# enordber/pepr

Measured on AMD Instinct MI355X. Metric: M site-lnL/sec (WAG+G4 full-tree likelihood evaluations x alignment patterns); the gene-trees/sec half of BASELINE.json's metric is search.gene_trees_per_sec, higher is better.
Workload: dtype f64

## Files before the change

__graft_entry__.py:

```python
import os
import subprocess
import sys

ROOT = os.path.dirname(os.path.abspath(__file__))
if ROOT not in sys.path:
    sys.path.insert(0, ROOT)


def build_jni_double():
    d = os.path.join(ROOT, "tests", "jni_double")
    subprocess.check_call(["gcc", "-O2", "-fPIC", "-shared", "-Wall", "-Werror", "-I" + d, os.path.join(ROOT, "bindings", "jni", "peprml_jni.c"),
                           os.path.join(d, "jni_double.c"), "-L" + os.path.join(ROOT, "pepr_amd"), "-lpeprml",
                           "-Wl,-rpath," + os.path.join(ROOT, "pepr_amd"), "-o", os.path.join(d, "libjni_double.so")])


def build_kernel_harness():
    d = os.path.join(ROOT, "tests", "kernel_harness")
    rocm = os.environ.get("ROCM_PATH", "/opt/rocm")
    subprocess.check_call(["g++", "-O1", "-std=c++17", "-fPIC", "-shared", "-Wall", "-Werror", "-D__HIP_PLATFORM_AMD__", "-I" + os.path.join(rocm, "include"),
                           os.path.join(d, "kh.cpp"), "-L" + os.path.join(ROOT, "pepr_amd"), "-lpeprml", "-L" + os.path.join(rocm, "lib"), "-lamdhip64",
                           "-Wl,-rpath,$ORIGIN/../../pepr_amd", "-Wl,-rpath," + os.path.join(rocm, "lib"), "-o", os.path.join(d, "libkh.so")])


def build():
    subprocess.check_call(["make", "-s", "-C", os.path.join(ROOT, "pepr_amd", "csrc")])
    build_jni_double()
    build_kernel_harness()
    subprocess.check_call(["make", "-s", "-C", os.path.join(ROOT, "oracle")])
    try:
        head = subprocess.run(["git", "-C", ROOT, "rev-parse", "--short", "HEAD"], capture_output=True, text=True, timeout=10).stdout.strip()
        dirty = subprocess.run(["git", "-C", ROOT, "status", "--porcelain", "--untracked-files=no"], capture_output=True, text=True, timeout=10).stdout.strip()
        if head:
            with open(os.path.join(ROOT, "pepr_amd", "BUILD_COMMIT"), "w") as f:
                f.write(head + ("+dirty" if dirty else "") + "\n")
    except Exception:
        pass
    import pepr_amd
    from pepr_amd import _lib
    L = _lib.load()
    for s in _lib.SYMBOLS:
        assert hasattr(L, s), "missing symbol " + s


def smoke():
    import numpy as np
    from oracle import po
    from pepr_amd import engine, synth
    build_needed = not os.path.exists(os.path.join(ROOT, "pepr_amd", "libpeprml.so"))
    if build_needed:
        build()
    ctx = engine.Context(0)
    names, rows, nw = synth.simulate_alignment(12, 400, 7, missing_frac=0.2)
    r = ctx.score([(names, rows)], [nw], alpha=0.7, site_lnl=True)[0]
    a = po.Alignment(names, rows); t = po.Tree(nw, a); e = po.Engine(a, po.Model(0), 4, 0.7)
    ref, refs = e.site_lnl(t)
    assert abs(r["lnl"] - ref) < 1e-9 * abs(ref), (r["lnl"], ref)
    assert np.abs(r["site_lnl"] - refs).max() < 1e-9
    o = ctx.optimize([(names, rows)], [nw], alpha=1.0)[0]
    assert o["lnl"] >= r["lnl"] - 1e-6, (o["lnl"], r["lnl"])
    print("smoke ok: lnL %.6f (oracle %.6f), optimised %.6f alpha %.4f" % (r["lnl"], ref, o["lnl"], o["alpha"]))
    ctx.close()


if __name__ == "__main__":
    build()
    if len(sys.argv) > 1 and sys.argv[1] == "smoke":
        smoke()
```

pepr_amd/csrc/api.cpp:

```cpp
#include <algorithm>
#include <cstdlib>
#include <cstring>
#include <memory>
#include <new>
#include <thread>

#include "../../include/peprml.h"
#include "api_types.hpp"

using namespace pml;

static thread_local std::string g_err;

static std::mutex g_fp_mu; static unsigned g_fp_seen[16]; static int g_fp_n = 0;
void pml_fpguard::note(unsigned v) {
    v &= ~0x3Fu;
    std::lock_guard<std::mutex> lk(g_fp_mu);
    for (int i = 0; i < g_fp_n; ++i) if (g_fp_seen[i] == v) return;
    if (g_fp_n < 16) g_fp_seen[g_fp_n++] = v;
}

extern "C" {

const char *pml_version(void) { return "peprml 0.2 (gfx950)"; }
// ... 98 lines not shown
    if (!b || g < 0 || g >= (int)b->b.genes.size()) return PML_EINVAL;
    return b->b.genes[g].aln.npat;
}

#define LOCKED(b) std::lock_guard<std::mutex> lk((b)->owner->c.mu)
#define GUARD(expr)                                                                            \
    try { return (expr); }                                                                     \
    catch (const std::bad_alloc &) { return b->owner->c.fail(PML_ENOMEM, "host allocation failed"); } \
    catch (const std::exception &e) { return b->owner->c.fail(PML_EINVAL, e.what()); }

int pml_batch_score(pml_batch *b, double *lnl) {
    if (!b || !lnl) return PML_EINVAL;
    pml_fpguard fpg;
    LOCKED(b);
    GUARD(b->b.score(std::vector<char>(), lnl));
}
int pml_batch_score_stored(pml_batch *b, double *lnl) {
    if (!b || !lnl) return PML_EINVAL;
    pml_fpguard fpg;
    LOCKED(b);
    GUARD(b->b.score(std::vector<char>(), lnl, true));
}
int pml_batch_site_lnl(pml_batch *b, int g, double *out) {
    if (!b || !out || g < 0 || g >= (int)b->b.genes.size()) return PML_EINVAL;
    pml_fpguard fpg;
    LOCKED(b);
    GUARD(b->b.site_lnl(g, out));
}
int pml_batch_set_alpha(pml_batch *b, int g, double alpha) {
    if (!b || g >= (int)b->b.genes.size() || !(alpha > 0)) return PML_EINVAL;
    pml_fpguard fpg;
    LOCKED(b);
    if (g < 0) for (int i = 0; i < (int)b->b.genes.size(); ++i) b->b.set_alpha(i, alpha);
    else b->b.set_alpha(g, alpha);
    return PML_OK;
}
int pml_batch_root_derivs(pml_batch *b, double *lnl, double *d1, double *d2) {
    if (!b || !lnl || !d1 || !d2) return PML_EINVAL;
    pml_fpguard fpg;
    LOCKED(b);
    GUARD(b->b.root_derivs(lnl, d1, d2));
}
int pml_batch_optimize(pml_batch *b, const pml_search_opts *opts, double *lnl, double *alpha) {
    if (!b || !lnl) return PML_EINVAL;
    pml_fpguard fpg;
    LOCKED(b);
    const bool oa = opts ? opts->optimize_alpha != 0 : true;
    const double eps = (opts && opts->epsilon > 0) ? opts->epsilon : 1e-4;
    int rc;
    try { rc = b->b.optimize(oa, eps, lnl); }
    catch (const std::exception &e) { return b->owner->c.fail(PML_EINVAL, e.what()); }
    if (rc) return rc;
    if (alpha) for (size_t g = 0; g < b->b.genes.size(); ++g) alpha[g] = b->b.genes[g].alpha;
    return PML_OK;
}
int pml_batch_search(pml_batch *b, const pml_search_opts *opts, double *lnl, double *alpha) {
    if (!b || !lnl) return PML_EINVAL;
    pml_fpguard fpg;
    LOCKED(b);
    int rc;
    try { rc = opts ? b->b.set_constraints(opts->nconstraints, opts->constraint_ntax, opts->constraint_names, opts->constraint_rows) : 0;
          if (!rc) rc = b->b.search(opts ? opts->nni != 0 : true, opts ? opts->spr_radius : 0,
                           opts ? opts->optimize_alpha != 0 : true,
                           (opts && opts->epsilon > 0) ? opts->epsilon : 1e-3, lnl); }
    catch (const std::exception &e) { return b->owner->c.fail(PML_EINVAL, e.what()); }
    if (rc) return rc;
    if (alpha) for (size_t g = 0; g < b->b.genes.size(); ++g) alpha[g] = b->b.genes[g].alpha;
    return PML_OK;
}
int pml_batch_newick(pml_batch *b, int g, int digits, char **out) {
    if (!b || !out || g < 0 || g >= (int)b->b.genes.size()) return PML_EINVAL;
    pml_fpguard fpg;
    LOCKED(b);
    const Gene &G = b->b.genes[g];
    *out = dup_string(G.tree.newick(G.aln.names, digits));
    return *out ? PML_OK : PML_ENOMEM;
}

enum { OP_SCORE, OP_OPTIMIZE, OP_SEARCH };

static size_t gene_bytes_bound(const pml_alignment &a, bool score_only) {
    const size_t mp = ((size_t)std::max(a.nsites, 1) + 31) / 32 * 32, nt = (size_t)std::max(a.ntax, 3);
    const size_t slots = (score_only ? nt - 2 : 3 * (nt - 2)) + NSCRATCH + MAXTAIL;
    return slots * CLV_ROWS * ((mp + 127) / 128 * 128) * 8 + slots * mp * 4 + nt * mp + 64 * mp + (1 << 16);
}

static int oneshot_on(Ctx &c, int op, int n, const pml_alignment *alns, const char *const *newicks,
                      const pml_model *model, const pml_search_opts *opts, int flags, pml_result *const *out, int share) {
    pml_fpguard fpg;
    std::vector<std::string> pstart; std::vector<const char *> pnw;
    static_assert(sizeof(pml_alignment) == sizeof(pml_alignment_view), "alignment view layout");
    if (op == OP_SEARCH && opts && opts->seed != 0) {
        std::vector<int> idx;
        for (int i = 0; i < n; ++i) if (!newicks || !newicks[i]) idx.push_back(i);
        if (!idx.empty()) {
            std::vector<pml_alignment_view> views;
            for (int i : idx) views.push_back(pml_alignment_view{alns[i].ntax, alns[i].nsites, alns[i].names, alns[i].rows});
            std::vector<Tree> trees; std::vector<EncodedAlignment> enc; std::vector<long long> len; std::vector<int> moves;
            if (int prc = parsimony_batch(&c, (int)idx.size(), views.data(), opts->seed, 20, trees, enc, len, moves)) return prc;
            pstart.resize(n); pnw.assign(n, nullptr);
            for (int i = 0; i < n; ++i) if (newicks && newicks[i]) pnw[i] = newicks[i];
            for (size_t k = 0; k < idx.size(); ++k) { pstart[idx[k]] = trees[k].newick(enc[k].names, 6); pnw[idx[k]] = pstart[idx[k]].c_str(); }
            newicks = pnw.data();
        }
    }
    Batch b;
    struct Drop { Batch &b; ~Drop() { b.destroy(); } } drop{b};
    b.share = share;
    int rc;
    try {
        rc = b.create(&c, n, reinterpret_cast<const pml_alignment_view *>(alns), newicks, model ? model->pi_mode : PML_PI_RAXML_3DP,
                      model ? model->ncat : 4, model ? model->alpha : 1.0, op == OP_SCORE);
        if (rc) return rc;
        std::vector<double> lnl(n);
        if (op == OP_SCORE) rc = b.score(std::vector<char>(), lnl.data());
        else if (op == OP_OPTIMIZE)
            rc = b.optimize(opts ? opts->optimize_alpha != 0 : true, (opts && opts->epsilon > 0) ? opts->epsilon : 1e-4, lnl.data());
        else {
            rc = opts ? b.set_constraints(opts->nconstraints, opts->constraint_ntax, opts->constraint_names, opts->constraint_rows) : 0;
            if (!rc) rc = b.search(opts ? opts->nni != 0 : true, opts ? opts->spr_radius : 0, opts ? opts->optimize_alpha != 0 : true,
                                   (opts && opts->epsilon > 0) ? opts->epsilon : 1e-3, lnl.data());
        }
        for (int i = 0; i < n && !rc; ++i) {
            const Gene &G = b.genes[i];
            pml_result &r = *out[i];
            r.lnl = lnl[i]; r.alpha = G.alpha; r.tree_length = G.tree.length();
            r.npatterns = G.aln.npat; r.nsites = G.aln.nsites;
            r.newick = dup_string(G.tree.newick(G.aln.names, op == OP_SCORE ? 10 : 20));
            if (op == OP_SCORE && (flags & PML_WANT_SITE_LNL)) {
                r.site_lnl = (double *)std::malloc(sizeof(double) * (G.aln.nsites > 0 ? G.aln.nsites : 1));
                if (!r.site_lnl) rc = c.fail(PML_ENOMEM, "host allocation failed");
                else rc = b.site_lnl(i, r.site_lnl);
            }
        }
    } catch (const std::bad_alloc &) { rc = c.fail(PML_ENOMEM, "host allocation failed"); }
    catch (const std::exception &e) { rc = c.fail(PML_EINVAL, e.what()); }
    return rc;
}

static Ctx *worker_ctx(pml_ctx *ctx, int k) {
    while ((int)ctx->workers.size() <= k) {
        std::unique_ptr<Ctx> w(new Ctx());
        if (w->init_worker(ctx->c)) { ctx->c.last_error = w->last_error; return nullptr; }
        ctx->workers.push_back(std::move(w));
    }
    return ctx->workers[k].get();
}
static int search_groups(int n, const pml_alignment *alns) {
    static const int env = std::getenv("PML_GROUPS") ? std::atoi(std::getenv("PML_GROUPS")) : 0;
    int maxcols = 0;
    for (int i = 0; i < n; ++i) maxcols = std::max(maxcols, alns[i].nsites);
    const int tiles = (maxcols + 127) / 128;
    int g = env > 0 ? std::min(env, 8) : 2;
    if (env <= 0) { while (g > 1 && n / g < 32) --g; }
    if (!std::getenv("PML_GROUPS_FORCE")) { while (g > 1 && tiles * g > 32) --g; }
    return std::max(g, 1);
}

static int oneshot_chunk(pml_ctx *ctx, int op, int n, const pml_alignment *alns, const char *const *newicks,
                         const pml_model *model, const pml_search_opts *opts, int flags, pml_result *out) {
    const int G = (op == OP_SEARCH) ? search_groups(n, alns) : 1;
    if (G <= 1) {
        std::vector<pml_result *> outs(n);
        for (int i = 0; i < n; ++i) outs[i] = out + i;
        return oneshot_on(ctx->c, op, n, alns, newicks, model, opts, flags, outs.data(), 1);
    }
    for (int k = 0; k < G; ++k) if (!worker_ctx(ctx, k)) return PML_EDEVICE;
// ... 474 lines not shown
```

pepr_amd/csrc/engine.cpp:

```cpp
#include "engine.hpp"

#include <algorithm>
#include <atomic>
#include <chrono>
#include <cmath>
#include <thread>
#include <cstring>

namespace pml {

#define HIPCHK(expr)                                                                          \
    do {                                                                                      \
        hipError_t e_ = (expr);                                                               \
        if (e_ != hipSuccess)                                                                 \
            return ctx->fail(-5, std::string(#expr) + ": " + hipGetErrorString(e_));          \
    } while (0)

int Ctx::init(int dev, bool prof) {
    Ctx *ctx = this;
    int count = 0;
    if (hipGetDeviceCount(&count) != hipSuccess || count <= 0) return fail(-3, "no HIP device available");
    if (dev < 0 || dev >= count) return fail(-3, "device ordinal out of range");
    device = dev; profile = prof;
    HIPCHK(hipSetDevice(device));
// ... 37 lines not shown
}
static void fill_model_dev(const Model &m, ModelDev &h) {
    std::memcpy(h.eval, m.eval, sizeof h.eval);
    std::memcpy(h.U, m.U, sizeof h.U);
    std::memcpy(h.Uinv, m.Uinv, sizeof h.Uinv);
    std::memcpy(h.pi, m.pi, sizeof h.pi);
    for (int k = 0; k < NS; ++k) for (int j = 0; j < NS; ++j) h.UinvT[j * NS + k] = m.Uinv[k * NS + j];
}
const Matrix *Ctx::matrix_of(int pm) const {
    const Ctx &r = root ? *root : *this;
    if (pm < PM_REGISTERED || (size_t)(pm - PM_REGISTERED) / 2 >= r.matrices.size()) return nullptr;
    return &r.matrices[(size_t)(pm - PM_REGISTERED) / 2];
}
std::string Ctx::model_name(int pm) const {
    if (pm == 0) return "PROTGAMMAWAG";
    if (pm == 1) return "PROTGAMMAWAG (full-precision frequencies)";
    if (pm == 2) return "PROTGAMMAWAGF";
    if (pm == PM_GTR) return "PROTGAMMAGTR";
    const Matrix *m = matrix_of(pm);
    if (!m) return "model code " + std::to_string(pm);
    std::string n = "PROTGAMMA";
    for (char ch : m->name) n += (char)std::toupper((unsigned char)ch);
    return (pm & 1) ? n + "F" : n;
}
int Ctx::ensure_model(int pm) {
    Ctx *ctx = this;
    if (!valid_code(pm)) return fail(-1, "bad pi_mode " + std::to_string(pm) + " (not a built-in model and not a registered matrix)");
    if (model_per_gene(pm) || shared_of(pm)) return 0;
    Shared sh{pm, nullptr, nullptr};
    HIPCHK(hipSetDevice(device));
    HIPCHK(hipMalloc((void **)&sh.d_model, sizeof(ModelDev)));
    HIPCHK(hipMalloc((void **)&sh.d_eigfrags, sizeof(double) * 2 * PFRAG));
    if (const Matrix *M = matrix_of(pm)) {
        struct In { double exch[NEXCH], pi[NS]; ModelReq req; } h, *d = nullptr;
        std::memcpy(h.exch, M->exch, sizeof h.exch); std::memcpy(h.pi, M->pi, sizeof h.pi);
        HIPCHK(hipMalloc((void **)&d, sizeof(In)));
        h.req = ModelReq{d->exch, d->pi, sh.d_model, -1, 0.0};
        HIPCHK(hipMemcpy(d, &h, sizeof h, hipMemcpyHostToDevice));
        Ev ev = tic_self(K_MODEL, sizeof(ModelDev));
        launch_model_build(&d->req, 1, stream, ev.a, ev.b);
        if (int rc = sync(stream)) return rc;
        HIPCHK(hipFree(d));
    } else {
        Model m; m.init(pm);
        ModelDev h;
        fill_model_dev(m, h);
        HIPCHK(hipMemcpy(sh.d_model, &h, sizeof h, hipMemcpyHostToDevice));
    }
    launch_eigfrags(sh.d_model, sh.d_eigfrags, stream);
    if (int rc = sync(stream)) return rc;
    HIPCHK(hipGetLastError());
    shared.push_back(sh);
    return 0;
}

int Batch::alloc_gene_models() {
    const size_t n = genes.size();
    HIPCHK(hipMalloc((void **)&d_gmodel, n * sizeof(ModelDev)));
    HIPCHK(hipMalloc((void **)&d_geig, n * 2 * PFRAG * sizeof(double)));
    HIPCHK(hipMalloc((void **)&d_gexch, n * NEXCH * sizeof(double)));
    HIPCHK(hipMalloc((void **)&d_gpi, n * NS * sizeof(double)));
    HIPCHK(hipMalloc((void **)&d_mreq, n * sizeof(ModelReq)));
    HIPCHK(hipHostMalloc((void **)&h_gexch, n * NEXCH * sizeof(double), hipHostMallocDefault));
    HIPCHK(hipHostMalloc((void **)&h_gpi, n * NS * sizeof(double), hipHostMallocDefault));
    HIPCHK(hipHostMalloc((void **)&h_mreq, n * sizeof(ModelReq), hipHostMallocDefault));
    return 0;
}
void Batch::empirical_pi(int g, double *pi) const {
    if (genes[g].counted_pi.empty()) empirical_freqs(genes[g].aln, pi);
    else std::memcpy(pi, genes[g].counted_pi.data(), sizeof(double) * NS);
}
void Batch::matrix_for(int g, double *exch, double *pi) const {
    const int code = genes[g].model_code;
    const Matrix *M = ctx->matrix_of(code);
    std::memcpy(exch, M ? M->exch : wag_exch(), sizeof(double) * NEXCH);
    if (code == PM_GTR) { const double last = exch[NEXCH - 1]; for (int i = 0; i < NEXCH; ++i) exch[i] /= last; }
    if (model_per_gene(code)) empirical_pi(g, pi);
    else std::memcpy(pi, M ? M->pi : wag_pi(code), sizeof(double) * NS);
    double sum = 0;
    for (int i = 0; i < NS; ++i) sum += pi[i];
    for (int i = 0; i < NS; ++i) pi[i] /= sum;
}
int Batch::build_gene_models() {
    const int n = (int)genes.size();
    if (int rc = alloc_gene_models()) return rc;
    std::vector<ModelDev> h(n);
    std::vector<int> dev;
    for (int g = 0; g < n; ++g) {
        const int code = genes[g].model_code;
        if (code == 2) {
            double pi[NS];
            empirical_pi(g, pi);
            Model m; m.init_pi(pi);
            fill_model_dev(m, h[g]);
            std::memcpy(h_gexch + (size_t)g * NEXCH, wag_exch(), sizeof(double) * NEXCH); std::memcpy(h_gpi + (size_t)g * NS, m.pi, sizeof m.pi);
            HIPCHK(hipMemcpyAsync(d_gmodel + g, &h[g], sizeof(ModelDev), hipMemcpyHostToDevice, ctx->stream));
            continue;
        }
        matrix_for(g, h_gexch + (size_t)g * NEXCH, h_gpi + (size_t)g * NS);
        if (model_per_gene(code)) { dev.push_back(g); continue; }
        if (int rc = ctx->ensure_model(code)) return rc;
        HIPCHK(hipMemcpyAsync(d_gmodel + g, ctx->shared_of(code)->d_model, sizeof(ModelDev), hipMemcpyDeviceToDevice, ctx->stream));
    }
    HIPCHK(hipMemcpyAsync(d_gexch, h_gexch, (size_t)n * NEXCH * sizeof(double), hipMemcpyHostToDevice, ctx->stream));
    HIPCHK(hipMemcpyAsync(d_gpi, h_gpi, (size_t)n * NS * sizeof(double), hipMemcpyHostToDevice, ctx->stream));
    if (int rc = build_models(dev, -1, nullptr)) return rc;
    if (dev.empty()) launch_eigfrags_n(d_gmodel, d_geig, n, ctx->stream);
    if (int rc = ctx->sync(ctx->stream)) return rc;
    HIPCHK(hipGetLastError());
    return 0;
}
int Batch::build_models(const std::vector<int> &gs, int patch, const double *vals) {
    if (gs.empty()) return 0;
    static const bool host_arm = std::getenv("PML_MODEL_HOST") != nullptr;
    const int n = (int)genes.size(), m = (int)gs.size();
    if (host_arm) {
        if (!h_gmodel) HIPCHK(hipHostMalloc((void **)&h_gmodel, (size_t)n * sizeof(ModelDev), hipHostMallocDefault));
        for (int i = 0; i < m; ++i) {
            const int g = gs[i];
            double ex[NEXCH];
            std::memcpy(ex, h_gexch + (size_t)g * NEXCH, sizeof ex);
            if (patch >= 0) ex[patch] = vals[i];
            Model md; md.init(ex, h_gpi + (size_t)g * NS);
            fill_model_dev(md, h_gmodel[g]);
            HIPCHK(hipMemcpyAsync(d_gmodel + g, h_gmodel + g, sizeof(ModelDev), hipMemcpyHostToDevice, ctx->stream));
        }
    } else {
        for (int i = 0; i < m; ++i) {
            const int g = gs[i];
            h_mreq[i] = ModelReq{d_gexch + (size_t)g * NEXCH, d_gpi + (size_t)g * NS, d_gmodel + g, patch, patch >= 0 ? vals[i] : 0.0};
        }
        HIPCHK(hipMemcpyAsync(d_mreq, h_mreq, (size_t)m * sizeof(ModelReq), hipMemcpyHostToDevice, ctx->stream));
        Ctx::Ev ev = ctx->tic_self(K_MODEL, (double)m * sizeof(ModelDev));
        launch_model_build(d_mreq, m, ctx->stream, ev.a, ev.b);
    }
    launch_eigfrags_n(d_gmodel, d_geig, n, ctx->stream);
    return 0;
}
int Batch::set_matrix(int g, const double *exch, const double *pi) {
    const int n = (int)genes.size();
    HIPCHK(hipSetDevice(ctx->device));
    if (!d_gmodel) {
        if (int rc = alloc_gene_models()) return rc;
        for (int i = 0; i < n; ++i) {
            matrix_for(i, h_gexch + (size_t)i * NEXCH, h_gpi + (size_t)i * NS);
            HIPCHK(hipMemcpyAsync(d_gmodel + i, d_shared, sizeof(ModelDev), hipMemcpyDeviceToDevice, ctx->stream));
            HIPCHK(hipMemcpyAsync(d_geig + (size_t)i * 2 * PFRAG, d_shared_eig, sizeof(double) * 2 * PFRAG, hipMemcpyDeviceToDevice, ctx->stream));
        }
        plan.valid = false;
    }
    std::vector<int> gs;
    for (int i = 0; i < n; ++i) if (g < 0 || i == g) gs.push_back(i);
    for (int i : gs) {
        std::memcpy(h_gexch + (size_t)i * NEXCH, exch, sizeof(double) * NEXCH);
        if (pi) {
            double sum = 0;
            for (int k = 0; k < NS; ++k) sum += pi[k];
            for (int k = 0; k < NS; ++k) h_gpi[(size_t)i * NS + k] = pi[k] / sum;
        }
        invalidate_all(i);
    }
    HIPCHK(hipMemcpyAsync(d_gexch, h_gexch, (size_t)n * NEXCH * sizeof(double), hipMemcpyHostToDevice, ctx->stream));
    HIPCHK(hipMemcpyAsync(d_gpi, h_gpi, (size_t)n * NS * sizeof(double), hipMemcpyHostToDevice, ctx->stream));
    if (int rc = build_models(gs, -1, nullptr)) return rc;
    if (int rc = ctx->sync(ctx->stream)) return rc;
    HIPCHK(hipGetLastError());
    return 0;
}
int Batch::get_matrix(int g, double *exch, double *pi) const {
    if (h_gexch) {
        if (exch) std::memcpy(exch, h_gexch + (size_t)g * NEXCH, sizeof(double) * NEXCH);
        if (pi) std::memcpy(pi, h_gpi + (size_t)g * NS, sizeof(double) * NS);
        return 0;
    }
    double ex[NEXCH], p[NS];
    matrix_for(g, ex, p);
    if (exch) std::memcpy(exch, ex, sizeof ex);
    if (pi) std::memcpy(pi, p, sizeof p);
    return 0;
}
hipEvent_t Ctx::get_event() {
    if (!pool.empty()) { hipEvent_t e = pool.back(); pool.pop_back(); return e; }
    hipEvent_t e; hipEventCreate(&e); return e;
}
void Ctx::tic(int kind, double bytes, double flops) {
    stats[kind].launches++; stats[kind].bytes += bytes; stats[kind].flops += flops;
    if (!profile) return;
    Ev ev{kind, get_event(), get_event()};
    hipEventRecord(ev.a, tic_stream ? tic_stream : stream);
    pending.push_back(ev);
}
void Ctx::toc() {
    if (!profile) return;
    hipEventRecord(pending.back().b, tic_stream ? tic_stream : stream);
}
Ctx::Ev Ctx::tic_self(int kind, double bytes, double flops) {
    stats[kind].launches++; stats[kind].bytes += bytes; stats[kind].flops += flops;
    if (!profile) return Ev{kind, nullptr, nullptr};
    pending.push_back(Ev{kind, get_event(), get_event()});
    return pending.back();
}
void Ctx::resolve_events() {
    for (auto &e : pending) {
        float ms = 0;
        if (hipEventElapsedTime(&ms, e.a, e.b) == hipSuccess) stats[e.kind].ms += ms;
        pool.push_back(e.a); pool.push_back(e.b);
    }
    pending.clear();
}

static size_t align_up(size_t x, size_t a) { return (x + a - 1) / a * a; }

struct DetRec { int batch, ntax, npat, nsites, kind, a, b, pad; double x, y, z; };
static std::vector<DetRec> *g_det = nullptr;
static std::mutex g_det_mu;
static bool det_on() {
    static const bool on = [] {
        const char *p = std::getenv("PML_DET_LOG");
        if (!p) return false;
        g_det = new std::vector<DetRec>(); g_det->reserve(1 << 22);
        std::atexit([] {
            const char *q = std::getenv("PML_DET_LOG"); FILE *f = q ? std::fopen(q, "w") : nullptr;
            if (!f) return;
            for (const DetRec &r : *g_det) std::fprintf(f, "B%d g%d_%d_%d %c %d %d %a %a %a\n", r.batch, r.ntax, r.npat, r.nsites, (char)r.kind, r.a, r.b, r.x, r.y, r.z);
            std::fclose(f);
        });
        return true;
    }();
    return on;
}
void det_record(int batch, const Gene &G, char kind, int a, int b, double x, double y, double z) {
    if (!det_on()) return;
    std::lock_guard<std::mutex> lk(g_det_mu);
    g_det->push_back(DetRec{batch, G.aln.ntax, G.aln.npat, G.aln.nsites, kind, a, b, 0, x, y, z});
}
static std::atomic<int> g_batch_id{0};
static double now_ms();

int Batch::create(Ctx *c, int n, const pml_alignment_view *alns, const char *const *newicks, int pm, int nc,
                  double alpha, bool score_only, const int *gene_codes) {
    ctx = c; pi_mode = pm; ncat = nc; score_only_batch = score_only;
    det_id = ++g_batch_id;
    virtual_cherries = std::getenv("PML_NO_CHERRY") == nullptr;
    virtual_pitch = virtual_cherries && std::getenv("PML_NO_PITCH") == nullptr;
    if (n <= 0) return ctx->fail(-1, "empty batch");
    if (nc != 1 && nc != 4) return ctx->fail(-1, "ncat must be 1 or 4");
    if (gene_codes) { for (int g = 0; g < n; ++g) if (!ctx->valid_code(gene_codes[g])) return ctx->fail(-1, "bad pi_mode " + std::to_string(gene_codes[g])); }
    else if (int rc = ctx->ensure_model(pm)) return rc;
    const bool per_gene = gene_codes != nullptr || model_per_gene(pm);
    if (!per_gene) { d_shared = ctx->shared_of(pm)->d_model; d_shared_eig = ctx->shared_of(pm)->d_eigfrags; }
    HIPCHK(hipSetDevice(ctx->device));
    genes.resize(n);
    for (int g = 0; g < n; ++g) genes[g].model_code = gene_codes ? gene_codes[g] : pm;
    const double t_create0 = now_ms();
    {
        const int nthreads = std::max(1, std::min({n, 16, (int)std::thread::hardware_concurrency()}));
        std::vector<std::string> errs(n);
        std::atomic<int> next{0};
        auto work = [&]() {
            for (int g = next++; g < n; g = next++) {
                Gene &G = genes[g];
                try {
                    if (!G.aln.encode(alns[g].ntax, alns[g].nsites, alns[g].names, alns[g].rows, errs[g])) continue;
                    if (newicks && newicks[g]) { if (!Tree::parse(newicks[g], G.aln.names, G.tree, errs[g])) continue; }
                    else G.tree = nj_tree(G.aln);
                } catch (const std::exception &e) { errs[g] = e.what(); }
            }
        };
        std::vector<std::thread> pool;
        for (int t = 1; t < nthreads; ++t) pool.emplace_back(work);
        work();
        for (auto &t : pool) t.join();
        for (int g = 0; g < n; ++g) if (!errs[g].empty()) return ctx->fail(-2, "gene " + std::to_string(g) + ": " + errs[g]);
    }
    if (std::getenv("PML_TRACE")) fprintf(stderr, "[pml] create: encode + start trees of %d genes %.1f ms\n", n, now_ms() - t_create0);
    if (int rc = layout(alpha, score_only)) return rc;
    return per_gene ? build_gene_models() : 0;
}

int Batch::layout(double alpha, bool score_only) {
    const int n = (int)genes.size();
    size_t total = 0;
    std::vector<size_t> off(n);
    for (int g = 0; g < n; ++g) {
        Gene &G = genes[g];
        const int nt = G.aln.ntax, mp = G.aln.mpad, ndir = 3 * (nt - 2);
        G.slot_cap = score_only ? (nt - 2) : ndir;
        G.slot_of.assign(ndir, -1); G.valid.assign(ndir, 0); G.pend_level.assign(ndir, -1);
        G.mark_all();
        off[g] = total;
        total += align_up((size_t)nt * mp, 256);
        total += align_up((size_t)mp * 8, 256);
        total += (size_t)(G.slot_cap + NSCRATCH) * clv_doubles(mp) * 8;
        total += align_up((size_t)(G.slot_cap + NSCRATCH) * mp * 4, 256);
        total += (size_t)MAXTAIL * clv_doubles(mp) * 8;
        total += (size_t)MAXTAIL * align_up((size_t)mp * 4, 256);
        total += (size_t)MAXTAIL * align_up((size_t)mp * 8, 256);
    }
    arena_bytes = total;
    const double t_alloc0 = now_ms();
    if (ctx->arena_cache && ctx->arena_cache_bytes >= total) {
        arena = ctx->arena_cache; arena_bytes = ctx->arena_cache_bytes;
        ctx->arena_cache = nullptr; ctx->arena_cache_bytes = 0;
    } else {
        if (ctx->arena_cache) { hipFree(ctx->arena_cache); ctx->arena_cache = nullptr; ctx->arena_cache_bytes = 0; }
        if (hipMalloc((void **)&arena, total) != hipSuccess) {
            arena = nullptr;
            return ctx->fail(-4, "device arena of " + std::to_string(total >> 20) + " MiB does not fit");
        }
    }
    if (std::getenv("PML_POISON_ARENA")) HIPCHK(hipMemsetAsync(arena, 0xFF, total, ctx->stream));
    for (int g = 0; g < n; ++g) {
        Gene &G = genes[g];
        const int nt = G.aln.ntax, mp = G.aln.mpad;
        char *p = arena + off[g];
        G.d_codes = (uint8_t *)p; p += align_up((size_t)nt * mp, 256);
        G.d_weight = (double *)p; p += align_up((size_t)mp * 8, 256);
        G.d_clv = (double *)p; p += (size_t)(G.slot_cap + NSCRATCH) * clv_doubles(mp) * 8;
        G.d_scl = (int *)p; p += align_up((size_t)(G.slot_cap + NSCRATCH) * mp * 4, 256);
        for (int k = 0; k < MAXTAIL; ++k) { G.d_sumtab[k] = (double *)p; p += clv_doubles(mp) * 8; }
        for (int k = 0; k < MAXTAIL; ++k) { G.d_sumscl[k] = (int *)p; p += align_up((size_t)mp * 4, 256); }
        for (int k = 0; k < MAXTAIL; ++k) { G.d_patlnl[k] = (double *)p; p += align_up((size_t)mp * 8, 256); }
        if (!G.aln.codes.empty()) {
            HIPCHK(hipMemcpyAsync(G.d_codes, G.aln.codes.data(), (size_t)nt * mp, hipMemcpyHostToDevice, ctx->stream));
            HIPCHK(hipMemcpyAsync(G.d_weight, G.aln.weight.data(), (size_t)mp * 8, hipMemcpyHostToDevice, ctx->stream));
        }
        set_alpha(g, alpha);
    }
    scalars_doubles = (size_t)8 * MAXTAIL * n;
    HIPCHK(hipMalloc((void **)&d_scalars, sizeof(double) * scalars_doubles));
    HIPCHK(hipHostMalloc((void **)&h_scalars, sizeof(double) * scalars_doubles, hipHostMallocDefault));
    std::memset(h_scalars, 0, sizeof(double) * scalars_doubles);
    HIPCHK(hipHostMalloc((void **)&h_plan_lnl, sizeof(double) * n, hipHostMallocMapped | hipHostMallocCoherent));
    HIPCHK(hipHostGetDevicePointer((void **)&d_plan_lnl, h_plan_lnl, 0));
    { if (int rc_ = ctx->sync(ctx->stream)) return rc_; }
    if (std::getenv("PML_TRACE")) fprintf(stderr, "[pml] layout: arena %.1f GiB allocated + uploaded in %.1f ms\n", (double)total / (1 << 30), now_ms() - t_alloc0);
    return 0;
}

void Batch::destroy() {
    if (!ctx) return;
    hipSetDevice(ctx->device);
    if (arena) {
        if (ctx->arena_cache_bytes < arena_bytes) {
            if (ctx->arena_cache) hipFree(ctx->arena_cache);
            ctx->arena_cache = arena; ctx->arena_cache_bytes = arena_bytes;
        } else hipFree(arena);
    }
    if (h_stage) hipHostFree(h_stage);
    if (d_stage) hipFree(d_stage);
    if (d_frags) hipFree(d_frags);
    if (d_nsync) hipFree(d_nsync);
    if (d_nctl) {
        if (std::getenv("PML_TRACE")) {
            NewtonCtl h[2];
            if (hipMemcpy(h, d_nctl, sizeof h, hipMemcpyDeviceToHost) == hipSuccess && h[0].n_requests)
                fprintf(stderr, "[pml] branch Newton: %llu requests, %.2f evaluations each\n", h[0].n_requests, (double)h[0].n_evals / (double)h[0].n_requests);
        }
        hipFree(d_nctl); d_nctl = nullptr;
    }
    if (d_gmodel) { hipFree(d_gmodel); d_gmodel = nullptr; }
    if (d_geig) { hipFree(d_geig); d_geig = nullptr; }
    if (d_gexch) { hipFree(d_gexch); d_gexch = nullptr; }
    if (d_gpi) { hipFree(d_gpi); d_gpi = nullptr; }
    if (d_mreq) { hipFree(d_mreq); d_mreq = nullptr; }
    if (h_gexch) { hipHostFree(h_gexch); h_gexch = nullptr; }
    if (h_gpi) { hipHostFree(h_gpi); h_gpi = nullptr; }
    if (h_mreq) { hipHostFree(h_mreq); h_mreq = nullptr; }
    if (h_gmodel) { hipHostFree(h_gmodel); h_gmodel = nullptr; }
    if (ev_stagger) { hipEventDestroy(ev_stagger); ev_stagger = nullptr; }
    if (d_nsync2) hipFree(d_nsync2);
    if (d_frags2) hipFree(d_frags2);
    d_nsync = d_nsync2 = nullptr; d_frags2 = nullptr; nsync_cap = nsync_cap2 = 0; frag_cap2 = 0;
    if (plan.h) hipHostFree(plan.h);
    if (plan.d) hipFree(plan.d);
    plan = Plan();
    if (h_scalars) hipHostFree(h_scalars);
    if (d_scalars) hipFree(d_scalars);
    if (h_plan_lnl) hipHostFree(h_plan_lnl);
    h_plan_lnl = d_plan_lnl = nullptr;
    if (h_chain) hipHostFree(h_chain);
    if (d_chain) hipFree(d_chain);
    if (d_lenpool) hipFree(d_lenpool);
    if (d_tailpool) { hipFree(d_tailpool); d_tailpool = nullptr; tailpool_cap = 0; }
    if (d_site2pat) { hipFree(d_site2pat); d_site2pat = nullptr; }
    h_chain = d_chain = nullptr; d_lenpool = nullptr; chain_cap = 0;
    arena = nullptr; h_stage = d_stage = nullptr; d_frags = nullptr; d_scalars = h_scalars = nullptr;
}

int GeneStore::create(Ctx *c, int n, const pml_alignment_view *alns) {
    ctx = c;
    HIPCHK(hipSetDevice(ctx->device));
    items.resize(n);
    std::vector<std::string> errs(n);
    std::atomic<int> next{0};
    auto work = [&]() {
        for (int g = next++; g < n; g = next++) {
            try { if (items[g].aln.encode(alns[g].ntax, alns[g].nsites, alns[g].names, alns[g].rows, errs[g])) pair_counts(items[g].aln, items[g].cmp, items[g].diff); }
            catch (const std::exception &e) { errs[g] = e.what(); }
        }
    };
    const int nthreads = std::max(1, std::min({n, 16, (int)std::thread::hardware_concurrency()}));
    std::vector<std::thread> pool;
    for (int t = 1; t < nthreads; ++t) pool.emplace_back(work);
    work();
    for (auto &t : pool) t.join();
    for (int g = 0; g < n; ++g) if (!errs[g].empty()) return ctx->fail(-2, "gene " + std::to_string(g) + ": " + errs[g]);
    size_t total = 0;
    for (auto &it : items) total += align_up((size_t)it.aln.ntax * it.aln.mpad, 256) + align_up((size_t)it.aln.mpad * 8, 256);
    if (hipMalloc((void **)&arena, total) != hipSuccess) { arena = nullptr; return ctx->fail(-4, "gene store does not fit on the device"); }
    char *p = arena;
    for (auto &it : items) {
        it.d_codes = (uint8_t *)p; p += align_up((size_t)it.aln.ntax * it.aln.mpad, 256);
        it.d_w = (double *)p; p += align_up((size_t)it.aln.mpad * 8, 256);
        HIPCHK(hipMemcpyAsync(it.d_codes, it.aln.codes.data(), (size_t)it.aln.ntax * it.aln.mpad, hipMemcpyHostToDevice, ctx->stream));
        HIPCHK(hipMemcpyAsync(it.d_w, it.aln.weight.data(), (size_t)it.aln.mpad * 8, hipMemcpyHostToDevice, ctx->stream));
    }
    { if (int rc_ = ctx->sync(ctx->stream)) return rc_; }
    return 0;
}
void GeneStore::destroy() { if (arena) { hipSetDevice(ctx->device); hipFree(arena); arena = nullptr; } items.clear(); }

int Batch::create_replicates(Ctx *c, const GeneStore &store, const std::vector<std::vector<int>> &sel, int pm, int nc, double alpha) {
    ctx = c; pi_mode = pm; ncat = nc; score_only_batch = false;
    virtual_cherries = std::getenv("PML_NO_CHERRY") == nullptr;
    virtual_pitch = virtual_cherries && std::getenv("PML_NO_PITCH") == nullptr;
    const int n = (int)sel.size();
    if (n <= 0) return ctx->fail(-1, "empty batch");
    if (int rc = ctx->ensure_model(pm)) return rc;
    const bool per_gene = model_per_gene(pm);
    if (!per_gene) { d_shared = ctx->shared_of(pm)->d_model; d_shared_eig = ctx->shared_of(pm)->d_eigfrags; }
    HIPCHK(hipSetDevice(ctx->device));
    genes.resize(n);
    for (auto &G : genes) G.model_code = pm;
    struct SegH { int rep, gene, off; size_t rowmap_off; };
    std::vector<SegH> segs; std::vector<int> rowmaps;
    int max_npat = 0;
    for (int r = 0; r < n; ++r) {
        Gene &G = genes[r]; EncodedAlignment &A = G.aln;
        std::vector<std::string> names;
// ... 223 lines not shown
    Gene &G = genes[g];
    const int nt = G.aln.ntax;
    if (v < nt || virt_kind(g, v, to)) return 0;
    {
        const int idx0 = (v - nt) * 3 + G.tree.slot(v, to);
        if (G.valid[idx0]) return 0;
        if (G.pend_level[idx0] >= 0) return G.pend_level[idx0];
    }
    struct Frame { int v, to, k, stage, lv[2]; };
    std::vector<Frame> st;
    st.reserve(64);
    st.push_back({v, to, G.tree.slot(v, to), 0, {0, 0}});
    int ret = 0;
    while (!st.empty()) {
        Frame &f = st.back();
        const int idx = (f.v - nt) * 3 + f.k;
        if (f.stage == 0) {
            if (G.valid[idx]) { ret = 0; st.pop_back(); continue; }
            if (G.pend_level[idx] >= 0) { ret = G.pend_level[idx]; st.pop_back(); continue; }
        }
        int ch[2], ci = 0;
        for (int q = 0; q < 3; ++q) if (q != f.k) ch[ci++] = G.tree.nbr[f.v][q];
        if (f.stage >= 1) f.lv[f.stage - 1] = ret;
        if (f.stage < 2) {
            const int c = ch[f.stage];
            f.stage++;
            if (c < nt || virt_kind(g, c, f.v)) { ret = 0; continue; }
            const int fv = f.v;
            st.push_back({c, fv, G.tree.slot(c, fv), 0, {0, 0}});
            continue;
        }
        const int lvl = std::max(f.lv[0], f.lv[1]) + 1;
        PendingOp op; op.gene = g; op.out_kind = SIDE_MSG; op.out_id = idx; op.level = lvl; ci = 0;
        for (int q = 0; q < 3; ++q) if (q != f.k) { op.child[ci] = msg(g, G.tree.nbr[f.v][q], f.v); op.t[ci] = G.tree.len[f.v][q]; ci++; }
        ops.push_back(op);
        G.pend_level[idx] = lvl;
        ret = lvl;
        st.pop_back();
    }
    return ret;
}

static double now_ms() {
    return std::chrono::duration<double, std::milli>(std::chrono::steady_clock::now().time_since_epoch()).count();
}

void Batch::newton_gave_up() {
    ++ctx->newton_giveups;
    if (std::getenv("PML_TRACE") && d_nctl) {
        NewtonCtl h[2];
        if (hipMemcpy(h, d_nctl, sizeof h, hipMemcpyDeviceToHost) == hipSuccess)
            fprintf(stderr, "[pml] k_newton exchange gave up: slice %d of %d, evaluation %d, arrived mask %08x%08x, tickets taken in its partition %d, (left * 1024 + partition) %d; tickets %d %d done %d %d oticket %d %d %d %d %d %d %d %d odone %d\n",
                    h[0].dbg[1], h[0].dbg[2], h[0].dbg[3], (unsigned)h[0].dbg[5], (unsigned)h[0].dbg[4], (unsigned)h[0].dbg[6], h[0].dbg[7], h[0].ticket[0], h[0].ticket[1], h[0].done[0], h[0].done[1],
                    h[0].oticket[0], h[0].oticket[1], h[0].oticket[2], h[0].oticket[3], h[0].oticket[4], h[0].oticket[5], h[0].oticket[6], h[0].oticket[7], h[0].odone);
        hipMemset(&d_nctl[0].dbg[0], 0, sizeof(int));
    }
    safe_left = safe_hold; safe_hold = std::min(safe_hold * 2, 1024);
}
int Batch::clear_abort() {
    if (!d_nctl) return 0;
    for (int l = 0; l < 2; ++l) HIPCHK(hipMemsetAsync(&d_nctl[l].abort, 0, sizeof(int), l ? ctx->stream2 : ctx->stream));
    { if (int rc_ = ctx->sync(ctx->stream2)) return rc_; }
    { if (int rc_ = ctx->sync(ctx->stream)) return rc_; }
    return 0;
}

int Batch::flush_deferred() {
    if (deferred.empty()) return 0;
    struct Guard { Batch *b; ~Guard() { b->deferred.clear(); b->ctx->tic_stream = nullptr; } } guard{this};
    const size_t lo = deferred.front().base, hi = deferred.back().base + deferred.back().bytes;
    const hipStream_t cs = deferred.front().lane ? ctx->stream2 : ctx->stream;
    HIPCHK(hipMemcpyAsync((char *)d_stage + lo, (char *)h_stage + lo, hi - lo, hipMemcpyHostToDevice, cs));
    const ModelDev *md = d_gmodel ? nullptr : d_shared;
    static const bool serialize = std::getenv("PML_SERIALIZE") != nullptr;
#define PML_SER() do { if (serialize) hipStreamSynchronize(st); } while (0)
    if (serialize) hipStreamSynchronize(cs);
    for (const Deferred &L : deferred) {
        const hipStream_t st = L.lane ? ctx->stream2 : ctx->stream;
        double *const frags_buf = L.lane ? d_frags2 : d_frags;
        char *ds = (char *)d_stage + L.base;
        ctx->tic_stream = st;
        if (L.nreq) {
            ctx->tic(K_PMAT, (double)L.nreq * PFRAG * 8);
            launch_pmat(md, (const PmatReq *)(ds + L.o_req), frags_buf, (int)L.nreq, st, d_gmodel != nullptr);
            ctx->toc(); PML_SER();
        }
        if (L.nruns) {
            ctx->tic(K_NEWVIEW, L.algo_bytes, L.algo_flops);
            launch_oplist((const NvOp *)(ds + L.o_ops), (const GeneRun *)(ds + L.o_runs), (int)L.nruns, L.max_mpad, L.any_pitch, L.any_chain, st, L.fused ? d_nctl + L.lane : nullptr);
            ctx->toc(); PML_SER();
        }
        if (L.stagger) hipEventRecord(ev_stagger, st);
        if (L.neval) {
            ctx->tic(K_REDUCE, 0);
            launch_reduce((const ReduceReq *)(ds + L.o_red), (int)L.neval, st);
            ctx->toc(); PML_SER();
        }
        if (L.nt_reg + L.nt_stream > 0) {
            ctx->tic(K_NEWTON, L.newton_bytes);
            if (L.seq) { launch_newton_seq(md, (const NewtonReq *)(ds + L.o_newt), (const int *)(ds + L.o_tick), L.nt_reg, L.nt_stream, d_nctl + L.lane, st); ++ctx->newton_seq_launches; }
            else launch_newton(md, (const NewtonReq *)(ds + L.o_newt), (const int *)(ds + L.o_tick), L.nt_reg, L.nt_stream, d_nctl + L.lane, st);
            ctx->toc(); PML_SER();
        }
        ctx->tic_stream = nullptr;
        if (hipError_t e = hipGetLastError(); e != hipSuccess) return ctx->fail(-5, std::string("kernel launch: ") + hipGetErrorString(e));
    }
#undef PML_SER
    flush_quota = std::min<size_t>(flush_quota * 2, 8);
    return 0;
}

int Batch::run(std::vector<PendingOp> &ops, const std::vector<Tail> &tails) {
    const double t_begin = now_ms();
    HIPCHK(hipSetDevice(ctx->device));
    std::stable_sort(ops.begin(), ops.end(), [](const PendingOp &a, const PendingOp &b) { return a.gene != b.gene ? a.gene < b.gene : a.part < b.part; });
    const size_t nops = ops.size(), ntail = tails.size();
    size_t neval = 0, nnewton = 0;
    for (auto &t : tails) { if (t.mode == MODE_EVALUATE) neval++; else if (t.mode != MODE_EVALUATE_CAT) nnewton++; }
    size_t nreq_max = 10 * nops + 9 * ntail;
    {
        std::vector<char> seen(genes.size(), 0);
        size_t keyed = 0, loose = 0;
        for (auto &o : ops) { if (!seen[o.gene]) { seen[o.gene] = 1; keyed += 5 * (size_t)genes[o.gene].aln.ntax; }
                              if (o.out_kind != SIDE_MSG) loose += (o.bv[0] < 0) + (o.bv[1] < 0); }
        for (auto &t : tails) { if (!seen[t.gene]) { seen[t.gene] = 1; keyed += 5 * (size_t)genes[t.gene].aln.ntax; }
                                if (t.mode >= MODE_EVALUATE && t.bv < 0) loose += 1; }
        nreq_max = std::min(nreq_max, keyed + loose);
    }
    bool any_pitch = false, any_chain = false;
    if (int rc = ensure_frags(std::max(nreq_max, (size_t)1))) return rc;
    double *&nsync_buf = lane ? d_nsync2 : d_nsync; size_t &nsync_c = lane ? nsync_cap2 : nsync_cap;
    if (nnewton > nsync_c) {
        if (chain) { if (int rc = chain_sync()) return rc; }
        if (nsync_buf) hipFree(nsync_buf);
        nsync_buf = nullptr; nsync_c = 0;
        const size_t cap = std::max(nnewton * 2, (size_t)256);
        HIPCHK(hipMalloc((void **)&nsync_buf, cap * NEWTON_SYNC_DOUBLES * sizeof(double)));
        HIPCHK(hipMemsetAsync(nsync_buf, 0, cap * NEWTON_SYNC_DOUBLES * sizeof(double), ctx->stream));
        { if (int rc_ = ctx->sync(ctx->stream)) return rc_; }
        nsync_c = cap;
    }
    if (nnewton && !d_nctl) {
        HIPCHK(hipMalloc((void **)&d_nctl, 2 * sizeof(NewtonCtl)));
        HIPCHK(hipMemsetAsync(d_nctl, 0, 2 * sizeof(NewtonCtl), ctx->stream));
        { if (int rc_ = ctx->sync(ctx->stream)) return rc_; }
    }
    const hipStream_t st = lane ? ctx->stream2 : ctx->stream;
    double *const frags_buf = lane ? d_frags2 : d_frags;
    ctx->tic_stream = st;
    const size_t ngenes = genes.size();
    std::vector<int> &nparts = run_nparts; nparts.assign(ngenes, 1);
    for (auto &o : ops) nparts[o.gene] = std::max(nparts[o.gene], o.part + 1);
    for (auto &t : tails) nparts[t.gene] = std::max(nparts[t.gene], t.part + 1);
    std::vector<size_t> &koff = run_koff; koff.assign(ngenes + 1, 0);
    for (size_t g = 0; g < ngenes; ++g) koff[g + 1] = koff[g] + (size_t)nparts[g];
    const size_t nkeys = koff[ngenes];
    const size_t o_req = 0;
    const size_t o_ops = align_up(o_req + nreq_max * sizeof(PmatReq), 256);
    const size_t o_runs = align_up(o_ops + (nops + ntail) * sizeof(NvOp), 256);
    const size_t o_red = align_up(o_runs + nkeys * sizeof(GeneRun), 256);
    const size_t o_newt = align_up(o_red + neval * sizeof(ReduceReq), 256);
    size_t ntick_max = 0;
    for (auto &t : tails) if (t.mode == MODE_SUMTABLE) ntick_max += (size_t)newton_split(genes[t.gene].aln.mpad);
    const size_t o_tick = align_up(o_newt + nnewton * sizeof(NewtonReq), 256);
    const size_t bytes = align_up(o_tick + ntick_max * sizeof(int), 256);
    if (chain && chain_off + bytes > h_cap) { if (int rc = chain_sync()) return rc; }
    if (int rc = ensure_stage(bytes)) return rc;
    const size_t base = chain ? chain_off : 0;
    if (chain) chain_off += bytes;
    char *hs = (char *)h_stage + base, *ds = (char *)d_stage + base;
    PmatReq *hreq = (PmatReq *)(hs + o_req);
    NvOp *hops = (NvOp *)(hs + o_ops);
    GeneRun *hruns = (GeneRun *)(hs + o_runs);
    ReduceReq *hred = (ReduceReq *)(hs + o_red);
    NewtonReq *hnewt = (NewtonReq *)(hs + o_newt);
    int *htick = (int *)(hs + o_tick);
    if (nnewton) ++newton_launch_seq;
    const unsigned tag_base = (newton_launch_seq & 0x3FFFFFu) << 10;
    static const bool fuse_env = std::getenv("PML_NO_FUSE") == nullptr && !(std::getenv("PML_CHAIN") && std::atoi(std::getenv("PML_CHAIN")) == 0);
    const bool fuse_ok = fuse_env && !newton_safe_mode();
    std::vector<char> fused_req(nnewton, 0);
    bool any_fused = false;
    std::vector<int> tail_req(ntail, -1);

    size_t nout = 0, nruns = 0, ie = 0, in = 0, ireq = 0, iop = 0;
    last_src.clear();
    int max_mpad = 0, newton_maxm = 0;
    double algo_bytes = 0, algo_flops = 0;
    bool req_ok = req_off.size() == genes.size() + 1;
    for (size_t g = 0; req_ok && g < genes.size(); ++g) req_ok = req_off[g + 1] - req_off[g] == (size_t)9 * genes[g].tree.nnodes();
    if (!req_ok) {
        req_off.assign(genes.size() + 1, 0);
        for (size_t g = 0; g < genes.size(); ++g) req_off[g + 1] = req_off[g] + (size_t)3 * 3 * genes[g].tree.nnodes();
        req_stamp.assign(req_off.back(), 0); req_ptr.assign(req_off.back(), nullptr); req_launch = 0;
        val_bucket.assign(genes.size() * 3, {}); val_stamp.assign(genes.size() * 3, 0);
    }
    if (++req_launch == 0) {
        std::fill(req_stamp.begin(), req_stamp.end(), 0u); std::fill(val_stamp.begin(), val_stamp.end(), 0u); req_launch = 1;
    }
    bool req_overflow = false;
    auto add_req = [&](size_t g, double t, int kind, int v, int q) -> const double * {
        uint64_t tbits = 0; size_t key = 0;
        std::vector<std::pair<uint64_t, const double *>> *bucket = nullptr;
        if (!record_plan) {
            if (v >= 0) {
                const Tree &T = genes[g].tree;
                const int w = T.nbr[v][q], a = v * 3 + q, b = w * 3 + T.slot(w, v);
                key = req_off[g] + (size_t)kind * 3 * T.nnodes() + (size_t)std::min(a, b);
                if (req_stamp[key] == req_launch) return req_ptr[key];
            } else {
                std::memcpy(&tbits, &t, 8);
                const size_t bi = g * 3 + (size_t)kind;
                if (val_stamp[bi] != req_launch) { val_bucket[bi].clear(); val_stamp[bi] = req_launch; }
                bucket = &val_bucket[bi];
                for (auto &e : *bucket) if (e.first == tbits) return e.second;
            }
        }
        if (ireq >= nreq_max) { req_overflow = true; return frags_buf; }
        PmatReq &r = hreq[ireq];
        r.t = t; std::memcpy(r.rates, genes[g].rates, sizeof r.rates); r.kind = kind; r.pad = 0;
        r.tp = (chain && v >= 0 && genes[g].len_pending[(size_t)v * 3 + q]) ? genes[g].d_len + (size_t)v * 3 + q : nullptr;
        r.md = d_gmodel ? d_gmodel + g : nullptr;
        last_src.push_back({(int)g, v, q, kind});
        const double *out = frags_buf + (ireq++) * FRAG_STRIDE;
        if (!record_plan) { if (v >= 0) { req_stamp[key] = req_launch; req_ptr[key] = out; } else bucket->push_back({tbits, out}); }
        return out;
    };
    struct Resolved { OpSide s; int kind; const int *scl; double bytes; double flops = 0; bool inner = true; };
    auto resolve = [&](size_t g, const Side &sd, Resolved &R) -> int {
        Gene &G = genes[g];
        const int mp = G.aln.mpad, nt = G.aln.ntax;
        R.s = OpSide{nullptr, nullptr, nullptr, nullptr, nullptr, nullptr, nullptr}; R.scl = nullptr;
        R.flops = 0; R.inner = true;
        if (sd.kind == SIDE_TIP) { R.kind = SK_TIP; R.s.p0 = G.d_codes + (size_t)sd.id * mp; R.bytes = 1; R.inner = false; return 0; }
        if (sd.kind == SIDE_CHERRY) {
            const int v = nt + sd.id / 3, k = sd.id % 3;
            int tips[2], qs[2], ci = 0;
            for (int q = 0; q < 3; ++q) if (q != k) { tips[ci] = G.tree.nbr[v][q]; qs[ci] = q; ++ci; }
            R.kind = SK_CHERRY;
            R.s.p0 = G.d_codes + (size_t)tips[0] * mp; R.s.p1 = G.d_codes + (size_t)tips[1] * mp;
            R.s.t0 = add_req(g, G.tree.len[v][qs[0]], PM_TIPTABLE, v, qs[0]);
            R.s.t1 = add_req(g, G.tree.len[v][qs[1]], PM_TIPTABLE, v, qs[1]);
            R.bytes = 640 + 642;
            R.flops = 80;
            return 0;
        }
        if (sd.kind == SIDE_PITCH) {
            const int X = nt + sd.id / 3, k = sd.id % 3;
            int qc = -1, qC = -1;
            for (int q = 0; q < 3; ++q) if (q != k) { if (G.tree.nbr[X][q] < nt) qc = q; else qC = q; }
            const int C = G.tree.nbr[X][qC], kC = G.tree.slot(C, X);
            int tips[2], qs[2], ci = 0;
            for (int q = 0; q < 3; ++q) if (q != kC) { tips[ci] = G.tree.nbr[C][q]; qs[ci] = q; ++ci; }
            R.kind = SK_PITCH;
            R.s.p0 = G.d_codes + (size_t)tips[0] * mp; R.s.p1 = G.d_codes + (size_t)tips[1] * mp;
            R.s.p2 = G.d_codes + (size_t)G.tree.nbr[X][qc] * mp;
            R.s.t0 = add_req(g, G.tree.len[C][qs[0]], PM_TIPTABLE, C, qs[0]);
            R.s.t1 = add_req(g, G.tree.len[C][qs[1]], PM_TIPTABLE, C, qs[1]);
            R.s.t2 = add_req(g, G.tree.len[X][qc], PM_TIPTABLE, X, qc);
            R.s.f = add_req(g, G.tree.len[X][qC], PM_FRAGS, X, qC);
            any_pitch = true;
            R.bytes = 640 + (640 + 642) + 1 + 640;
            R.flops = 80 + 3280;
            return 0;
        }
        const int slot = sd.kind == SIDE_MSG ? G.slot_of[sd.id] : G.slot_cap + sd.id;
        if (slot < 0) return -1;
        R.kind = SK_CLV; R.s.p0 = G.d_clv + (size_t)slot * clv_doubles(mp); R.scl = G.d_scl + (size_t)slot * mp; R.bytes = 640;
        return 0;
    };

    std::vector<std::vector<int>> &tails_of = run_tails_of;
    if (tails_of.size() < nkeys) tails_of.resize(nkeys);
    for (auto &v : tails_of) v.clear();
    for (size_t i = 0; i < ntail; ++i) {
        if (tails[i].slot < 0 || tails[i].slot >= MAXTAIL) return ctx->fail(-1, "internal: bad tail slot");
        tails_of[koff[tails[i].gene] + (size_t)tails[i].part].push_back((int)i);
    }
    for (size_t g = 0; g < ngenes; ++g) for (int part = 0; part < nparts[g]; ++part) {
        const size_t key = koff[g] + (size_t)part;
        const bool has_ops = iop < nops && ops[iop].gene == (int)g && ops[iop].part == part;
        if (!has_ops && tails_of[key].empty()) continue;
        Gene &G = genes[g];
        const int mp = G.aln.mpad;
        GeneRun &run = hruns[nruns++];
        run.op_begin = (int)nout;
        max_mpad = std::max(max_mpad, mp);
        static const int chain_env = std::getenv("PML_CHAIN") ? std::atoi(std::getenv("PML_CHAIN")) : 2;
        const bool chain_reads = chain_env == 2 || (chain_env == 1 && record_plan), chain_nostore = chain_env >= 1 && record_plan && !record_stored;
        long last_nv = -1, last_nv_op = -1;
        auto chained_from = [&](const Side &sd, int kind) {
            return chain_reads && last_nv >= 0 && kind == SK_CLV && sd.kind == ops[last_nv_op].out_kind && sd.id == ops[last_nv_op].out_id;
        };
        auto consume_last = [&]() {
            any_chain = true;
            if (chain_nostore || ops[last_nv_op].transient) { hops[last_nv].flags |= OPF_NO_STORE; ops[last_nv_op].unstored = true; }
        };
        auto emit_tail = [&](const Tail &t) -> int {
            NvOp &d = hops[nout++];
            std::memset(&d, 0, sizeof d);
            Resolved L, R;
            if (resolve(g, t.a, L) || resolve(g, t.b, R)) return ctx->fail(-5, "internal: tail message has no slot");
            d.l = L.s; d.r = R.s; d.l_scl = L.scl; d.r_scl = R.scl;
            d.flags = L.kind | (R.kind << 2); d.mpad = mp; d.mode = t.mode;
            if (chained_from(t.a, L.kind)) { d.flags |= OPF_CHAIN_L; consume_last(); }
            else if (t.mode >= MODE_EVALUATE && chained_from(t.b, R.kind)) { d.flags |= OPF_CHAIN_R; consume_last(); }
            double *result = t.result_dev ? t.result_dev : d_scalars + 8 * (g * MAXTAIL + t.slot);
            if (t.mode == MODE_EVALUATE_CAT) {
                if (!t.patlnl_dev || !t.scl_dev) return ctx->fail(-1, "internal: table slice missing");
                d.pl = d.pr = add_req(g, t.t0, PM_FRAGS_PI, t.bv, t.bq);
                d.out = t.patlnl_dev; d.out_scl = t.scl_dev;
                algo_bytes += (double)G.aln.npat * (L.bytes + R.bytes + 36);
                algo_flops += (double)G.aln.npat * (3360 + L.flops + R.flops);
            } else if (t.mode == MODE_EVALUATE) {
                d.pl = d.pr = add_req(g, t.t0, PM_FRAGS_PI, t.bv, t.bq);
                double *pl = t.patlnl_dev ? t.patlnl_dev : G.d_patlnl[t.slot];
                d.out = pl; d.out_scl = nullptr;
                ReduceReq &rr = hred[ie++];
                rr.patlnl = pl; rr.weight = G.d_weight; rr.out = result; rr.mpad = mp; rr.pad = 0;
                algo_bytes += (double)G.aln.npat * (L.bytes + R.bytes + 8);
                algo_flops += (double)G.aln.npat * (3360 + L.flops + R.flops);
            } else {
                d.pl = eig_of((int)g); d.pr = d.pl + PFRAG;
                double *stab = t.sumtab_dev ? t.sumtab_dev : G.d_sumtab[t.slot];
                int *sscl = t.sumtab_dev ? reinterpret_cast<int *>(t.sumtab_dev + clv_doubles(mp)) : G.d_sumscl[t.slot];
                d.out = stab; d.out_scl = sscl;
                NewtonReq &nr = hnewt[in];
                nr.md = model_of((int)g); nr.tag_base = tag_base; nr.pad0 = 0;
                if (fuse_ok && !t.patlnl_dev && newton_reg_form(mp)) {
                    d.flags |= OPF_FUSED_NEWTON; d.aux = (const NewtonReq *)(ds + o_newt) + in;
                    fused_req[in] = 1; any_fused = true; any_chain = true;
                }
                last_nv = -1; last_nv_op = -1;
                tail_req[&t - tails.data()] = (int)in;
                nr.ticket0 = 0; nr.pad = 0;
                nr.sumtab = stab; nr.weight = G.d_weight; nr.scl = sscl;
                std::memcpy(nr.rates, G.rates, sizeof nr.rates);
                nr.t0 = t.t0; nr.tol = newton_tol; nr.out = result; nr.mpad = mp; nr.max_iter = t.max_iter;
                nr.t_dev0 = t.t_dev0; nr.t_dev1 = t.t_dev1; nr.patlnl = t.patlnl_dev;
                nr.sync = nsync_buf + (size_t)in * NEWTON_SYNC_DOUBLES; newton_maxm = std::max(newton_maxm, mp);
                algo_bytes += (double)G.aln.npat * (L.bytes + R.bytes + 640);
                algo_flops += (double)G.aln.npat * (6480 + L.flops + R.flops);
                in++;
            }
            return 0;
        };
        size_t ti = 0; int emitted = 0;
        auto flush_tails = [&](bool all) -> int {
            while (ti < tails_of[key].size()) {
                const Tail &t = tails[tails_of[key][ti]];
                if (!all && (t.after < 0 || t.after > emitted)) break;
                if (int rc = emit_tail(t)) return rc;
                ++ti;
            }
            return 0;
        };
        if (int rc = flush_tails(false)) return rc;
        for (; iop < nops && ops[iop].gene == (int)g && ops[iop].part == part; ++iop) {
            PendingOp &o = ops[iop];
            const int s = o.out_kind == SIDE_MSG ? slot_for(G, o.out_id) : G.slot_cap + o.out_id;
            if (s < 0) return ctx->fail(-4, "CLV slots exhausted (score-only batch used for a multi-root request)");
            NvOp &d = hops[nout++];
            std::memset(&d, 0, sizeof d);
            d.mode = MODE_NEWVIEW;
            d.out = G.d_clv + (size_t)s * clv_doubles(mp);
            d.out_scl = G.d_scl + (size_t)s * mp;
            Resolved S[2];
            if (resolve(g, o.child[0], S[0]) || resolve(g, o.child[1], S[1])) return ctx->fail(-5, "internal: child message has no slot");
            d.mpad = mp;
            d.flags = S[0].kind | (S[1].kind << 2);
            const double *pm[2];
            for (int c = 0; c < 2; ++c) {
                int bv = o.bv[c], bq = o.bq[c];
                if (o.out_kind == SIDE_MSG) {
                    bv = G.aln.ntax + o.out_id / 3; const int k = o.out_id % 3;
                    int seen = 0;
                    for (bq = 0; bq < 3; ++bq) if (bq != k) { if (seen == c) break; ++seen; }
                }
                pm[c] = add_req(g, o.t[c], PM_FRAGS, bv, bq);
            }
            Side ch[2] = {o.child[0], o.child[1]};
            if (chained_from(ch[1], S[1].kind)) { std::swap(S[0], S[1]); std::swap(pm[0], pm[1]); std::swap(ch[0], ch[1]); }
            d.flags = S[0].kind | (S[1].kind << 2);
            if (chained_from(ch[0], S[0].kind)) { d.flags |= OPF_CHAIN_L; consume_last(); }
            d.l = S[0].s; d.r = S[1].s; d.l_scl = S[0].scl; d.r_scl = S[1].scl; d.pl = pm[0]; d.pr = pm[1];
            algo_bytes += (double)G.aln.npat * (S[0].bytes + S[1].bytes + 640);
            algo_flops += (double)G.aln.npat * ((S[0].inner && S[1].inner ? 6480 : (S[0].inner || S[1].inner ? 3280 : 80)) + S[0].flops + S[1].flops);
            last_nv = (long)nout - 1; last_nv_op = (long)iop;
            ++emitted;
            if (int rc = flush_tails(false)) return rc;
        }
        if (int rc = flush_tails(true)) return rc;
        run.op_end = (int)nout;
        if (mp <= 16 * TILE_PAT)
            for (int i = run.op_begin; i < run.op_end; ++i) if (hops[i].mode == MODE_NEWVIEW) hops[i].flags |= OPF_NT_STORE;
    }

    if (req_overflow) return ctx->fail(-5, "internal: transition-matrix request bound exceeded");
    int nt_reg = 0, nt_stream = 0;
    const bool seq_launch = nnewton > 0 && newton_safe_mode();
    {
        int cur = 0;
        for (int pass = 0; pass < 2; ++pass) {
            for (size_t i = 0; i < nnewton; ++i) {
                if (fused_req[i] || newton_reg_form(hnewt[i].mpad) != (pass == 0)) continue;
                const int S = seq_launch ? 1 : newton_split(hnewt[i].mpad);
                hnewt[i].ticket0 = cur - (pass == 0 ? 0 : nt_reg);
                for (int k = 0; k < S; ++k) htick[cur++] = (int)i;
            }
            if (pass == 0) nt_reg = cur; else nt_stream = cur - nt_reg;
        }
        if (nnewton && safe_left > 0 && !safe_now) --safe_left;
    }
    double newton_bytes = 0;
    for (size_t i = 0; i < ntail; ++i) if (tails[i].mode == MODE_SUMTABLE && !fused_req[tail_req[i]]) newton_bytes += (double)genes[tails[i].gene].aln.npat * 640;
    Deferred L;
    L.base = base; L.bytes = bytes; L.o_req = o_req; L.o_ops = o_ops; L.o_runs = o_runs; L.o_red = o_red; L.o_newt = o_newt;
    L.o_tick = o_tick; L.nt_reg = nt_reg; L.nt_stream = nt_stream; L.seq = seq_launch; L.fused = any_fused;
    L.nreq = ireq; L.nruns = nruns; L.neval = neval; L.nnewton = nnewton; L.max_mpad = max_mpad; L.newton_maxm = newton_maxm;
    L.any_pitch = any_pitch; L.any_chain = any_chain; L.algo_bytes = algo_bytes; L.algo_flops = algo_flops; L.newton_bytes = newton_bytes; L.lane = lane; L.stagger = record_stagger;
    record_stagger = false;
    deferred.push_back(L);
    const bool defer = chain && !lanes_active;
    if (!defer || deferred.size() >= flush_quota) { if (int rc = flush_deferred()) return rc; }
    ctx->tic_stream = nullptr;
    const double t_launched = now_ms();
    ctx->stats[K_HOST_BUILD].launches++; ctx->stats[K_HOST_BUILD].ms += t_launched - t_begin;
    if (!chain) {
        bool pooled = false;
        for (auto &t : tails) pooled = pooled || t.result_host != nullptr;
        if (int rc = fetch_results(pooled)) return rc;
        { if (int rc_ = ctx->sync(ctx->stream)) return rc_; }
        HIPCHK(hipGetLastError());
        const double t_done = now_ms();
        ctx->stats[K_HOST_WAIT].launches++; ctx->stats[K_HOST_WAIT].ms += t_done - t_launched;
        host_phase_ms[HP_RUN_SYNCED] += t_launched - t_begin;
        ctx->resolve_events();
        auto result_of = [&](const Tail &t) { return t.result_host ? t.result_host : (t.result_dev ? (const double *)nullptr : res(t.gene, t.slot)); };
        std::vector<int> bad;
        for (size_t i = 0; i < ntail; ++i) {
            const Tail &t = tails[i];
            if (t.mode != MODE_SUMTABLE) continue;
            const double *h = result_of(t);
            if (h && !std::isfinite(h[1])) bad.push_back(tail_req[i]);
        }
        bool bad_fused = false;
        for (int i : bad) bad_fused = bad_fused || fused_req[i];
        if (bad_fused && !in_retry) {
            newton_gave_up(); ctx->newton_reissued += (long long)bad.size();
            if (int rc = clear_abort()) return rc;
            for (auto &o : ops) { o.unstored = false; if (o.out_kind == SIDE_MSG) genes[o.gene].pend_level[o.out_id] = -1; }
            in_retry = true;
            const int rc = run(ops, tails);
            in_retry = false;
            return rc;
        }
        if (!bad.empty() && !seq_launch && !bad_fused) {
            newton_gave_up(); ctx->newton_reissued += (long long)bad.size();
            int nr = 0, ns = 0;
            for (int pass = 0; pass < 2; ++pass) for (int i : bad) if (newton_reg_form(hnewt[i].mpad) == (pass == 0)) { htick[nr + ns] = i; ++(pass == 0 ? nr : ns); }
            if (int rc = clear_abort()) return rc;
            HIPCHK(hipMemcpyAsync(ds + o_tick, hs + o_tick, bad.size() * sizeof(int), hipMemcpyHostToDevice, ctx->stream));
            launch_newton_seq(nullptr, (const NewtonReq *)(ds + o_newt), (const int *)(ds + o_tick), nr, ns, d_nctl + lane, ctx->stream);
            ++ctx->newton_seq_launches;
            if (int rc = fetch_results(pooled)) return rc;
            { if (int rc_ = ctx->sync(ctx->stream)) return rc_; }
            HIPCHK(hipGetLastError());
        }
        for (auto &t : tails) {
            if (t.mode == MODE_EVALUATE_CAT) continue;
            const double *h = result_of(t);
#ifndef ABL_KEEP_GOING
            if (h && !std::isfinite(t.mode == MODE_EVALUATE ? h[0] : h[1]))
                return ctx->fail(-5, t.mode == MODE_EVALUATE ? "device returned a non-finite likelihood" : "k_newton: non-finite branch likelihood (also from the no-exchange form)");
#endif
        }
    }
    for (auto &o : ops) if (o.out_kind == SIDE_MSG) { Gene &G = genes[o.gene]; G.valid[o.out_id] = o.unstored ? 0 : 1; G.pend_level[o.out_id] = -1; }
    if (record_plan) {
        record_plan = false;
        Plan &P = plan;
        if (P.bytes < bytes) {
            if (P.h) hipHostFree(P.h);
            if (P.d) hipFree(P.d);
            P.h = P.d = nullptr; P.bytes = 0;
            HIPCHK(hipHostMalloc(&P.h, bytes)); HIPCHK(hipMalloc(&P.d, bytes)); P.bytes = bytes;
        }
        std::memcpy(P.h, hs, bytes);
        HIPCHK(hipMemcpyAsync(P.d, ds, bytes, hipMemcpyDeviceToDevice, ctx->stream));
        ReduceReq *pred = (ReduceReq *)((char *)P.h + o_red);
        P.per_gene = neval == genes.size();
        for (size_t g = 0; P.per_gene && g < neval; ++g) P.per_gene = pred[g].out == d_scalars + 8 * (g * MAXTAIL);
        if (P.per_gene) {
            for (size_t g = 0; g < neval; ++g) pred[g].out = d_plan_lnl + g;
            HIPCHK(hipMemcpyAsync((char *)P.d + o_red, pred, neval * sizeof(ReduceReq), hipMemcpyHostToDevice, ctx->stream));
        }
        P.len_seen.assign(genes.size(), {});
        P.o_req = o_req; P.o_ops = o_ops; P.o_runs = o_runs; P.o_red = o_red;
        P.nreq = ireq; P.nruns = nruns; P.neval = neval; P.max_mpad = max_mpad; P.algo_bytes = algo_bytes; P.algo_flops = algo_flops; P.stored = record_stored; P.any_pitch = any_pitch; P.any_chain = any_chain;
        P.rates_seen.resize(genes.size()); for (size_t g = 0; g < genes.size(); ++g) P.rates_seen[g] = genes[g].rates_epoch;
        P.src = last_src; P.outs.clear();
// ... 87 lines not shown
}
int Batch::site_lnl(int g, double *out) {
    Gene &G = genes[g];
    if ((int)G.aln.site2pat.size() != G.aln.nsites) return ctx->fail(-1, "per-site lnL is not available for device-gathered replicates");
    std::vector<char> act(genes.size(), 0); act[g] = 1;
    std::vector<double> l(genes.size());
    if (int rc = evaluate(act, l.data())) return rc;
    std::vector<double> pat(G.aln.mpad);
    HIPCHK(hipMemcpy(pat.data(), G.d_patlnl[0], sizeof(double) * G.aln.mpad, hipMemcpyDeviceToHost));
    for (int s = 0; s < G.aln.nsites; ++s) out[s] = pat[G.aln.site2pat[s]];
    return 0;
}
int Batch::root_derivs(double *lnl, double *d1, double *d2) {
    std::vector<PendingOp> ops; std::vector<Tail> tails;
    for (int g = 0; g < (int)genes.size(); ++g) {
        Gene &G = genes[g];
        const int r = G.tree.nbr[0][0];
        need(g, r, 0, ops);
        tails.push_back({g, msg(g, 0, r), msg(g, r, 0), MODE_SUMTABLE, G.tree.len[0][0], 0});
    }
    if (int rc = run(ops, tails)) return rc;
    for (int g = 0; g < (int)genes.size(); ++g) { lnl[g] = res(g)[1]; d1[g] = res(g)[2]; d2[g] = res(g)[3]; }
    return 0;
}

int Batch::smooth_pass(const std::vector<char> &active, std::vector<double> &maxdelta, double thr) {
    const int n = (int)genes.size();
    maxdelta.assign(n, 0.0);
    struct SafeOff { bool &f; ~SafeOff() { f = false; } } safe_off{safe_now};
    double hp_t = now_ms();
    std::vector<std::vector<std::pair<int, int>>> &order = pass_order;
    std::vector<std::vector<uint8_t>> &next = pass_next;
    if ((int)order.size() != n) { order.assign(n, {}); next.assign(n, {}); }
    size_t maxlen = 0;
    struct F { int v, from, k; };
    std::vector<F> st; st.reserve(256);
    for (int g = 0; g < n; ++g) {
        order[g].clear();
        if (!active[g]) { next[g].clear(); continue; }
        Gene &G = genes[g];
        const Tree &T = G.tree; const int nt = T.ntax;
        if (G.dirty.size() != (size_t)T.nnodes() * 3) G.mark_all();
        next[g].assign((size_t)T.nnodes() * 3, 0);
        st.clear(); st.push_back({0, -1, 0});
        while (!st.empty()) {
            F &f = st.back();
            if (f.k >= 3) { st.pop_back(); continue; }
            const int k = f.k, w = T.nbr[f.v][k]; f.k++;
            if (w < 0 || w == f.from) continue;
            if (G.dirty[f.v * 3 + k]) order[g].push_back({f.v, w});
            if (w >= nt) { const int fv = f.v; st.push_back({w, fv, 0}); }
        }
        maxlen = std::max(maxlen, order[g].size());
    }
    ++cnt_passes;
    host_phase_ms[HP_PASS_SETUP] += now_ms() - hp_t; hp_t = now_ms();
    static const bool no_chain = std::getenv("PML_NO_CHAIN") != nullptr;
    size_t nres = 0; for (int g = 0; g < n; ++g) nres += order[g].size();
    struct Done { int gene, v, w; double old; size_t idx; };
    std::vector<Done> done; done.reserve(nres);
    for (int attempt = 0; attempt < 2; ++attempt) {
    done.clear();
    if (!no_chain) { if (int rc = chain_begin(nres)) return rc; }
    auto fail_out = [&](int rc) { if (chain) { chain_sync(); chain = false; } return rc; };
    static const bool lanes_on = std::getenv("PML_LANES") != nullptr;
    int nact = 0; for (int g = 0; g < n; ++g) nact += active[g] && !order[g].empty();
    const bool two_lanes = chain && lanes_on && nact >= 16;
    lanes_active = two_lanes;
    for (size_t step = 0; step < maxlen; ++step) {
        ++cnt_smooth;
        const size_t first = done.size();
        for (int ln = 0; ln < (two_lanes ? 2 : 1); ++ln) {
            std::vector<PendingOp> ops; std::vector<Tail> tails;
            for (int g = 0; g < n; ++g) {
                if (!active[g] || step >= order[g].size()) continue;
                if (two_lanes && (g & 1) != ln) continue;
                auto [v, w] = order[g][step];
                Gene &G = genes[g];
                need(g, v, w, ops); need(g, w, v, ops);
                Tail t{g, msg(g, v, w), msg(g, w, v), MODE_SUMTABLE, G.tree.len[v][G.tree.slot(v, w)], 32};
                if (chain) {
                    t.result_dev = d_chain + 4 * done.size();
                    t.t_dev0 = G.d_len + (size_t)v * 3 + G.tree.slot(v, w); t.t_dev1 = G.d_len + (size_t)w * 3 + G.tree.slot(w, v);
                }
                done.push_back({g, v, w, t.t0, done.size()});
                tails.push_back(t);
            }
            if (tails.empty()) continue;
            lane = ln;
            if (two_lanes && step == 0) {
                if (!ev_stagger) hipEventCreateWithFlags(&ev_stagger, hipEventDisableTiming);
                if (ln == 0) record_stagger = true;
                else hipStreamWaitEvent(ctx->stream2, ev_stagger, 0);
            }
            const int rc = run(ops, tails);
            lane = 0;
            if (rc) return fail_out(rc);
        }
        if (chain) {
            for (size_t i = first; i < done.size(); ++i) {
                Gene &G = genes[done[i].gene]; const int v = done[i].v, w = done[i].w;
                G.len_pending[(size_t)v * 3 + G.tree.slot(v, w)] = 1; G.len_pending[(size_t)w * 3 + G.tree.slot(w, v)] = 1;
                branch_changed(done[i].gene, v, w);
            }
        } else {
            for (size_t i = first; i < done.size(); ++i) {
                Gene &G = genes[done[i].gene]; const int v = done[i].v, w = done[i].w;
                const double nl = res(done[i].gene)[0], old = done[i].old, dl = std::fabs(nl - old);
                maxdelta[done[i].gene] = std::max(maxdelta[done[i].gene], dl);
                if (nl != old) { G.tree.set_len(v, w, nl); branch_changed(done[i].gene, v, w); }
                if (dl > thr) { std::swap(G.dirty, next[done[i].gene]); G.mark_node(v); G.mark_node(w); std::swap(G.dirty, next[done[i].gene]); }
            }
        }
    }
    host_phase_ms[HP_PASS_STEPS] += now_ms() - hp_t;
    if (chain) {
        const double t0 = now_ms();
        if (int rc = chain_sync()) { chain = false; return rc; }
        ctx->stats[K_HOST_WAIT].launches++; ctx->stats[K_HOST_WAIT].ms += now_ms() - t0;
        host_phase_ms[HP_PASS_SYNC] += now_ms() - t0; hp_t = now_ms();
        chain = false; lanes_active = false;
        bool gave_up = false;
        for (auto &d : done) gave_up = gave_up || !std::isfinite(h_chain[4 * d.idx + 1]);
        if (gave_up) {
            if (attempt == 1 || safe_now) return ctx->fail(-5, "k_newton: non-finite branch likelihood (also from the no-exchange form)");
            newton_gave_up(); ctx->newton_reissued += (long long)done.size();
            if (int rc = clear_abort()) return rc;
            for (int g = 0; g < n; ++g) if (active[g]) { std::fill(genes[g].len_pending.begin(), genes[g].len_pending.end(), 0); invalidate_all(g); }
            safe_now = true;
            continue;
        }
        for (auto &d : done) {
            Gene &G = genes[d.gene];
            const double nl = h_chain[4 * d.idx], dl = std::fabs(nl - d.old);
            det_record(det_id, G, 'S', d.v, d.w, d.old, nl, h_chain[4 * d.idx + 1]);
            maxdelta[d.gene] = std::max(maxdelta[d.gene], dl);
            G.tree.set_len(d.v, d.w, nl);
            if (dl > thr) { std::swap(G.dirty, next[d.gene]); G.mark_node(d.v); G.mark_node(d.w); std::swap(G.dirty, next[d.gene]); }
        }
        for (auto &G : genes) std::fill(G.len_pending.begin(), G.len_pending.end(), 0);
    }
    break;
    }
    safe_now = false;
    for (int g = 0; g < n; ++g) if (active[g]) genes[g].dirty.swap(next[g]);
    host_phase_ms[HP_PASS_POST] += now_ms() - hp_t;
    return 0;
}

int Batch::gamma20(std::vector<double> &lnl20, std::vector<double> &alpha20, std::vector<double> &rescale20) {
    const int n = (int)genes.size();
    HIPCHK(hipSetDevice(ctx->device));
    double rates[G20_RATES]; g20_rates(rates);
    std::vector<size_t> off(n); size_t bytes = 0;
    for (int g = 0; g < n; ++g) { off[g] = bytes; bytes += align_up((size_t)genes[g].aln.mpad * (G20_RATES * 8 + (G20_RATES / 4) * 4), 256); }
    if (int rc = ensure_tailpool(bytes)) return rc;
    auto table = [&](int g) { return reinterpret_cast<double *>(d_tailpool + off[g]); };
    auto counts = [&](int g) { return reinterpret_cast<int *>(d_tailpool + off[g] + (size_t)genes[g].aln.mpad * G20_RATES * 8); };
    struct RatesBack { Batch *b; ~RatesBack() { for (int g = 0; g < (int)b->genes.size(); ++g) b->set_alpha(g, b->genes[g].alpha); } };
    for (int j = 0; j < G20_RATES / 4; ++j) {
        RatesBack back{this};
        std::vector<PendingOp> ops; std::vector<Tail> tails;
        for (int g = 0; g < n; ++g) {
            Gene &G = genes[g];
            for (int c = 0; c < 4; ++c) G.rates[c] = rates[4 * j + c];
            ++G.rates_epoch; invalidate_all(g);
            const int r = G.tree.nbr[0][0];
            need(g, r, 0, ops);
            Tail t{g, msg(g, 0, r), msg(g, r, 0), MODE_EVALUATE_CAT, G.tree.len[0][0], 0, 0, -1, 0, 0};
            t.patlnl_dev = table(g) + (size_t)4 * j * G.aln.mpad; t.scl_dev = counts(g) + (size_t)j * G.aln.mpad;
            tails.push_back(t);
        }
        if (int rc = run(ops, tails)) return rc;
    }
    if (int rc = ensure_results((size_t)n)) return rc;
    if (int rc = ensure_stage((size_t)n * sizeof(G20Req))) return rc;
    std::vector<double> la(n, 0.0), lm(n, 0.0), f(n, 0.0);
    auto objective = [&](const std::vector<char> &act) -> int {
        G20Req *h = (G20Req *)h_stage; int k = 0;
        std::vector<int> who;
        for (int g = 0; g < n; ++g) {
            if (!act[g]) continue;
            G20Req &r = h[k++];
            r.table = table(g); r.cnt = counts(g); r.weight = genes[g].d_weight; r.out = d_chain + 4 * g; r.patlnl = nullptr;
            r.mpad = genes[g].aln.mpad; r.pad = 0;
            g20_weights(std::exp(la[g]), std::exp(lm[g]), r.w);
            who.push_back(g);
        }
        if (!k) return 0;
        HIPCHK(hipMemcpyAsync(d_stage, h_stage, (size_t)k * sizeof(G20Req), hipMemcpyHostToDevice, ctx->stream));
        launch_g20((const G20Req *)d_stage, k, ctx->stream);
        results_used = (size_t)n;
        if (int rc = fetch_results(true)) return rc;
        { if (int rc_ = ctx->sync(ctx->stream)) return rc_; }
        HIPCHK(hipGetLastError());
        for (int g : who) { f[g] = -h_chain[4 * g]; if (!std::isfinite(f[g])) return ctx->fail(-5, "device returned a non-finite Gamma20 likelihood"); }
        return 0;
    };
    std::vector<char> all(n, 1), active(n, 1);
    if (int rc = objective(all)) return rc;
    const double LO = std::log(0.01), HI = std::log(10.0), TOL = 1e-3;
    for (int round = 0; round < 10; ++round) {
        bool any = false; for (char a : active) any |= a;
        if (!any) break;
        const std::vector<double> start(f);
        for (int which = 0; which < 2; ++which) {
            std::vector<double> &x = which ? lm : la;
            std::vector<Brent> br(n);
            std::vector<char> act(active);
            for (int g = 0; g < n; ++g) if (act[g]) br[g].start(LO, HI, x[g], f[g], TOL);
            for (;;) {
                bool moved = false;
                for (int g = 0; g < n; ++g) { if (!act[g]) continue; if (br[g].propose()) { x[g] = br[g].u; moved = true; } else act[g] = 0; }
                if (!moved) break;
                if (int rc = objective(act)) return rc;
                for (int g = 0; g < n; ++g) if (act[g]) br[g].update(f[g]);
            }
            for (int g = 0; g < n; ++g) if (active[g]) { x[g] = br[g].x; f[g] = br[g].fx; }
        }
        for (int g = 0; g < n; ++g) if (active[g] && !(f[g] < start[g] - 1e-3)) active[g] = 0;
// ... 137 lines not shown
```

pepr_amd/csrc/engine.hpp:

```cpp
#pragma once
#include <hip/hip_runtime.h>

#include <array>
#include <mutex>
#include <string>
#include <vector>

#include "host.hpp"
#include "kernels.h"

namespace pml {

constexpr int MAXTAIL = 4;

enum { K_PMAT = 0, K_NEWVIEW = 1, K_EVALUATE = 2, K_SUMTABLE = 3, K_NEWTON = 4, K_REDUCE = 5, K_HOST_BUILD = 6, K_HOST_WAIT = 7, K_MODEL = 8, K_CODEHIST = 9, K_COUNT = 10 };

enum { PM_GTR = 3, PM_REGISTERED = 16 };
inline bool model_per_gene(int pm) { return pm == 2 || pm == PM_GTR || (pm >= PM_REGISTERED && (pm & 1)); }
constexpr double RATE_MIN = 1e-7, RATE_MAX = 1e6;
struct Matrix { std::string name; double exch[NEXCH]; double pi[NS]; };

struct Ctx {
    int device = 0;
    bool profile = false;
    hipStream_t stream = nullptr;
    hipStream_t stream2 = nullptr;
    std::mutex mu;
    std::string last_error;
    struct Shared { int code; ModelDev *d_model; double *d_eigfrags; };
    std::vector<Shared> shared;
    const Shared *shared_of(int pm) const { for (auto &m : shared) if (m.code == pm) return &m; return nullptr; }
    const Ctx *root = nullptr;
    std::vector<Matrix> matrices;
    const Matrix *matrix_of(int pm) const;
    bool valid_code(int pm) const { return (pm >= 0 && pm <= PM_GTR) || matrix_of(pm) != nullptr; }
    std::string model_name(int pm) const;
    struct KStat { long long launches = 0; double ms = 0; double bytes = 0; double flops = 0; } stats[K_COUNT];
    long long newton_giveups = 0, newton_reissued = 0, newton_seq_launches = 0;
    struct Ev { int kind; hipEvent_t a, b; };
    std::vector<Ev> pending;
    std::vector<hipEvent_t> pool;
    char *arena_cache = nullptr; size_t arena_cache_bytes = 0;

    int init(int dev, bool prof);
    int init_worker(const Ctx &parent);
    bool owns_stream = true;
    hipEvent_t ev_sync = nullptr;
    int sync(hipStream_t s);
    void destroy();
    int ensure_model(int pi_mode);
    hipEvent_t get_event();
    hipStream_t tic_stream = nullptr;
    void tic(int kind, double bytes, double flops = 0);
    void toc();
    Ev tic_self(int kind, double bytes, double flops = 0);
    void resolve_events();
    int fail(int code, const std::string &msg) { last_error = msg; return code; }
};

struct Gene {
    EncodedAlignment aln;
    Tree tree;
    double alpha = 1.0;
    double rates[NCAT] = {1, 1, 1, 1};
    unsigned rates_epoch = 0;
    int model_code = 0;
    std::vector<long long> code_hist; std::vector<double> counted_pi;
    uint8_t *d_codes = nullptr;
    double *d_weight = nullptr;
    double *d_clv = nullptr;
    int *d_scl = nullptr;
    double *d_sumtab[MAXTAIL] = {};
    int *d_sumscl[MAXTAIL] = {};
    double *d_patlnl[MAXTAIL] = {};
    int slot_cap = 0, next_slot = 0;
    std::vector<int> slot_of;
    std::vector<uint8_t> valid;
    std::vector<int> pend_level;
    std::vector<Constraint> cons;
    std::vector<uint8_t> dirty;
    double *d_len = nullptr;
    std::vector<uint8_t> len_pending;
    void mark_node(int v) { for (int k = 0; k < 3; ++k) { const int w = tree.nbr[v][k]; if (w < 0) continue; dirty[v * 3 + k] = 1; dirty[w * 3 + tree.slot(w, v)] = 1; } }
    void mark_all() { dirty.assign((size_t)tree.nnodes() * 3, 1); }
    void mark_none() { dirty.assign((size_t)tree.nnodes() * 3, 0); }
};

void det_record(int batch, const Gene &G, char kind, int a, int b, double x, double y, double z);

struct pml_alignment_view { int ntax, nsites; const char *const *names; const char *const *rows; };

struct GeneStore {
    struct Item { EncodedAlignment aln; std::vector<int64_t> cmp, diff; uint8_t *d_codes = nullptr; double *d_w = nullptr; };
    Ctx *ctx = nullptr; std::vector<Item> items; char *arena = nullptr;
    int create(Ctx *c, int n, const pml_alignment_view *alns);
    void destroy();
};

constexpr int NNI_PARTS = 6;
constexpr int NSCRATCH = 4 * NNI_PARTS > 8 ? 4 * NNI_PARTS : 8;
enum { SIDE_TIP = 0, SIDE_MSG = 1, SIDE_SCRATCH = 2, SIDE_CHERRY = 3, SIDE_PITCH = 4 };
struct Side { int kind, id; };
struct PendingOp { int gene, out_kind, out_id, level; Side child[2]; double t[2]; int bv[2] = {-1, -1}, bq[2] = {0, 0};
                   bool unstored = false;
                   bool transient = false;
                   int part = 0;  };

struct Batch {
    Ctx *ctx = nullptr;
    int pi_mode = 0, ncat = 4, det_id = 0;
    const ModelDev *d_shared = nullptr; const double *d_shared_eig = nullptr;
    ModelDev *d_gmodel = nullptr; double *d_geig = nullptr;
    double *d_gexch = nullptr, *d_gpi = nullptr, *h_gexch = nullptr, *h_gpi = nullptr;
    ModelReq *d_mreq = nullptr, *h_mreq = nullptr;
    ModelDev *h_gmodel = nullptr;
    const ModelDev *model_of(int g) const { return d_gmodel ? d_gmodel + g : d_shared; }
    const double *eig_of(int g) const { return d_geig ? d_geig + (size_t)g * 2 * PFRAG : d_shared_eig; }
    int alloc_gene_models();
    int build_gene_models();
    void matrix_for(int g, double *exch190, double *pi20) const;
    void empirical_pi(int g, double *pi20) const;
    int count_replicate_freqs();
    int build_models(const std::vector<int> &gs, int patch, const double *vals);
    int set_matrix(int g , const double *exch190, const double *pi20 );
    int get_matrix(int g, double *exch190, double *pi20) const;
    int opt_rates(const std::vector<char> &active, double *lnl, double tol);
    bool rates_on = true;
    long cnt_rate_trials = 0;
    int share = 1;
    double newton_tol = 1e-8;
    std::vector<Gene> genes;
    char *arena = nullptr; size_t arena_bytes = 0;
    void *h_stage = nullptr; size_t h_cap = 0;
    void *d_stage = nullptr; size_t d_cap = 0;
    double *d_frags = nullptr; size_t frag_cap = 0;
    double *d_frags2 = nullptr; size_t frag_cap2 = 0;
    double *d_nsync2 = nullptr; size_t nsync_cap2 = 0;
    int lane = 0;
    hipEvent_t ev_stagger = nullptr; bool record_stagger = false;
    double *d_scalars = nullptr; double *h_scalars = nullptr;
    size_t scalars_doubles = 0, results_used = 0;
    double *h_plan_lnl = nullptr, *d_plan_lnl = nullptr;
    int fetch_results(bool pooled);
    double *d_nsync = nullptr; size_t nsync_cap = 0;
    NewtonCtl *d_nctl = nullptr;
    int safe_left = 0, safe_hold = 4; bool safe_now = false;
    unsigned newton_launch_seq = 0;
    bool in_retry = false;
    bool newton_safe_mode() { return safe_now || safe_left > 0; }
    void newton_gave_up();
    int clear_abort();
    struct ReqSrc { int gene, v, q, fold; };
    struct Plan {
        bool valid = false; unsigned epoch = 0;
        void *h = nullptr, *d = nullptr; size_t bytes = 0;
        size_t o_req = 0, o_ops = 0, o_runs = 0, o_red = 0, nreq = 0, nruns = 0, neval = 0;
        int max_mpad = 0; double algo_bytes = 0, algo_flops = 0; bool any_pitch = false, any_chain = false;
        bool stored = false;
        std::vector<ReqSrc> src; std::vector<std::pair<int, int>> outs;
        std::vector<unsigned> rates_seen;
        std::vector<std::vector<std::array<double, 3>>> len_seen;
        std::vector<char> moved;
        bool per_gene = false;
    } plan;
    long cnt_smooth = 0, cnt_nni = 0, cnt_spr = 0, cnt_eval = 0, cnt_passes = 0;
    enum { HP_PASS_SETUP, HP_PASS_STEPS, HP_PASS_SYNC, HP_PASS_POST, HP_NNI_BUILD, HP_NNI_RUN, HP_NNI_SELECT, HP_ALPHA_HOST, HP_RUN_SYNCED, HP_N };
    double host_phase_ms[HP_N] = {0};
    unsigned topo_epoch = 0;
    bool score_only_batch = false;
    int replay_plan(double *lnl);
    bool record_plan = false, record_stored = false;
    std::vector<ReqSrc> last_src;
    std::vector<size_t> req_off; std::vector<uint32_t> req_stamp; std::vector<const double *> req_ptr; uint32_t req_launch = 0;
    std::vector<std::vector<int>> run_tails_of; std::vector<int> run_nparts; std::vector<size_t> run_koff;
    std::vector<std::vector<std::pair<int, int>>> pass_order; std::vector<std::vector<uint8_t>> pass_next;
    std::vector<std::vector<std::pair<uint64_t, const double *>>> val_bucket; std::vector<uint32_t> val_stamp;
    bool chain = false; size_t chain_off = 0;
    double *d_lenpool = nullptr;
    double *d_chain = nullptr, *h_chain = nullptr; size_t chain_cap = 0;
    struct Deferred { size_t base, bytes, o_req, o_ops, o_runs, o_red, o_newt, o_tick, nreq, nruns, neval, nnewton; int nt_reg, nt_stream; bool seq, fused;
                      int max_mpad, newton_maxm, lane; bool any_pitch, any_chain, stagger; double algo_bytes, newton_bytes, algo_flops; };
    std::vector<Deferred> deferred; size_t flush_quota = 1; bool lanes_active = false;
    int flush_deferred();
    int chain_begin(size_t nresults);
    int ensure_results(size_t nresults);
    char *d_tailpool = nullptr; size_t tailpool_cap = 0;
    int ensure_tailpool(size_t bytes);
    int chain_sync();

    int create(Ctx *c, int n, const pml_alignment_view *alns, const char *const *newicks,
               int pi_mode, int ncat, double alpha, bool score_only, const int *gene_codes = nullptr );
    int create_replicates(Ctx *c, const GeneStore &store, const std::vector<std::vector<int>> &sel, int pi_mode, int ncat, double alpha);
    int layout(double alpha, bool score_only);
    void destroy();

    void set_alpha(int g, double alpha);
    void invalidate_all(int g);
    void branch_changed(int g, int a, int b);
    int evaluate(const std::vector<char> &active, double *lnl);
    int score(const std::vector<char> &active, double *lnl, bool stored = false);
    int site_lnl(int g, double *out);
    int root_derivs(double *lnl, double *d1, double *d2);
    int smooth_pass(const std::vector<char> &active, std::vector<double> &maxdelta, double thr);
    int opt_alpha(const std::vector<char> &active, double *lnl, double tol = 1e-4);
    int optimize(bool opt_alpha_flag, double eps, double *lnl, const std::vector<char> *mask = nullptr);
    int light_smooth(const std::vector<char> &active, double *lnl);
    int nni_round(const std::vector<char> &active, std::vector<double> &lnl, std::vector<int> &applied);
    int spr_round(const std::vector<char> &active, int radius, std::vector<double> &lnl, std::vector<int> &moves);
    int search(bool nni, int spr_radius, bool opt_alpha_flag, double eps, double *lnl);
    int gamma20(std::vector<double> &lnl20, std::vector<double> &alpha20, std::vector<double> &rescale20);
    int sh_support(int nboot, unsigned long long seed, std::vector<std::vector<double>> &support, std::vector<std::vector<std::pair<int, int>>> &edges_out);
    int *d_site2pat = nullptr; std::vector<size_t> site2pat_off;
    int set_constraints(int ncons, int ntax, const char *const *names, const char *const *rows);

    int need(int g, int v, int to, std::vector<PendingOp> &ops);
    struct Tail { int gene; Side a, b; int mode; double t0; int max_iter; int slot = 0; int after = -1;
                  int bv = -1, bq = 0;
                  double *result_dev = nullptr;
                  double *t_dev0 = nullptr, *t_dev1 = nullptr;
                  double *patlnl_dev = nullptr;
                  double *sumtab_dev = nullptr;
                  int *scl_dev = nullptr;
                  const double *result_host = nullptr;
                  int part = 0;                                };
    double *res(int g, int slot = 0) const { return h_scalars + 8 * ((size_t)g * MAXTAIL + slot); }
    Side msg(int g, int node, int toward) const;
    bool is_cherry(int g, int node, int toward) const;
    int virt_kind(int g, int node, int toward) const;
    bool virtual_pitch = true;
    bool virtual_cherries = true;
    int run(std::vector<PendingOp> &ops, const std::vector<Tail> &tails);
    int ensure_stage(size_t bytes);
    int ensure_frags(size_t sets);
    int slot_for(Gene &g, int idx);
};

int parsimony_batch(Ctx *ctx, int n, const pml_alignment_view *alns, unsigned seed, int radius, std::vector<Tree> &trees_out,
                    std::vector<EncodedAlignment> &alns_out, std::vector<long long> &lengths_out, std::vector<int> &moves_out);

}
```

pepr_amd/csrc/kernels.h:

```cpp
#pragma once
#include <hip/hip_runtime.h>
#include <cstdint>

namespace pml {

constexpr int NS = 20;
constexpr int NCAT = 4;
constexpr int CLV_ROWS = NCAT * NS;
constexpr int PFRAG = NCAT * 25 * 16;
constexpr int PAT_PER_WAVE = 32;
constexpr int TILE_PAT = 128;
constexpr size_t clv_doubles(int mpad) { return (size_t)((mpad + TILE_PAT - 1) / TILE_PAT) * TILE_PAT * (NCAT * NS); }
constexpr size_t clv_index(int row, int p) { return ((size_t)(p >> 7) * (NCAT * NS) + (size_t)row) * TILE_PAT + (size_t)(p & (TILE_PAT - 1)); }
constexpr int NCODES = 23;
constexpr int TIPTAB_KK = 6;
constexpr int TIPTAB_DOUBLES = NCAT * NCODES * 4 * TIPTAB_KK;
constexpr int FRAG_STRIDE = TIPTAB_DOUBLES;

struct ModelDev {
    double eval[NS];
    double U[NS * NS];
    double Uinv[NS * NS];
    double pi[NS];
    double UinvT[NS * NS];
};

struct ModelReq {
    const double *exch;
    const double *pi;
    ModelDev *out;
    int patch;
    double patch_val;
};
constexpr int NEXCH = NS * (NS - 1) / 2;

struct PmatReq {
    double t;
    double rates[NCAT];
    int kind;
    int pad;
    const double *tp;
    const ModelDev *md;
};
enum { PM_FRAGS = 0, PM_FRAGS_PI = 1, PM_TIPTABLE = 2 };

enum { SK_CLV = 0, SK_TIP = 1, SK_CHERRY = 2, SK_PITCH = 3 };
constexpr int OPF_NT_STORE = 16;
constexpr int OPF_CHAIN_L = 32, OPF_CHAIN_R = 64, OPF_NO_STORE = 128;
constexpr int OPF_FUSED_NEWTON = 256;
struct OpSide {
    const void *p0, *p1, *p2;
    const double *t0, *t1, *t2;
    const double *f;
};

struct NvOp {
    double *out;
    OpSide l, r;
    int *out_scl;
    const int *l_scl;
    const int *r_scl;
    const double *pl;
    const double *pr;
    int mpad;
    int flags;
    int mode;
    int pad;
    const void *aux;
};
static_assert(sizeof(NvOp) == 184, "NvOp layout");

struct GeneRun {
    int op_begin, op_end;
};

struct ReduceReq {
    const double *patlnl;
    const double *weight;
    double *out;
    int mpad;
    int pad;
};

struct NewtonReq {
    const double *sumtab;
    const double *weight;
    const int *scl;
    double rates[NCAT];
    double t0;
    double tol;
    double *out;
    double *sync;
    const ModelDev *md;
    unsigned tag_base;
    unsigned pad0;
    double *t_dev0, *t_dev1;
    double *patlnl;
    int mpad;
    int max_iter;
    int ticket0;
    int pad;
};
constexpr int NEWTON_MAX_SPLIT = 64;
constexpr int NEWTON_SLICE_PAT = 128;
__host__ __device__ constexpr int newton_split(int mpad) { return (mpad + NEWTON_SLICE_PAT - 1) / NEWTON_SLICE_PAT < NEWTON_MAX_SPLIT ? ((mpad + NEWTON_SLICE_PAT - 1) / NEWTON_SLICE_PAT < 1 ? 1 : (mpad + NEWTON_SLICE_PAT - 1) / NEWTON_SLICE_PAT) : NEWTON_MAX_SPLIT; }
__host__ __device__ constexpr int newton_slice(int mpad) { return mpad <= NEWTON_SLICE_PAT * NEWTON_MAX_SPLIT ? NEWTON_SLICE_PAT : ((mpad / 32 + newton_split(mpad) - 1) / newton_split(mpad)) * 32; }
__host__ __device__ constexpr bool newton_reg_form(int mpad) { return newton_slice(mpad) <= NEWTON_SLICE_PAT; }
struct NewtonCtl { int ticket[2]; int done[2]; int abort; int odone; int pad[2]; int oticket[8]; int dbg[8];
                   unsigned long long n_requests, n_evals; };
constexpr int NEWTON_SYNC_DOUBLES = 2 * NEWTON_MAX_SPLIT * 6;

enum { MODE_NEWVIEW = 0, MODE_SUMTABLE = 1, MODE_EVALUATE = 2, MODE_EVALUATE_CAT = 3 };

constexpr int G20_RATES = 20;
struct G20Req {
    const double *table;
    const int *cnt;
    const double *weight;
    double w[G20_RATES];
    double *out;
    double *patlnl;
    int mpad, pad;
};
void launch_g20(const G20Req *reqs, int n, hipStream_t s);

struct GatherSeg {
    const uint8_t *src; const double *w; uint8_t *dst; double *dst_w; const int *rowmap;
    int src_mpad, npat, dst_mpad, dst_off, ntax_dst, pad;
};
void launch_gather(const GatherSeg *segs, int nsegs, int max_npat, hipStream_t s);
struct CodeHistReq { const uint8_t *codes; const double *weight; int ntax, mpad; };
void launch_codehist(const CodeHistReq *reqs, int nreqs, int max_mpad, long long *out, hipStream_t s);

struct ShReq { const double *l0, *l1, *l2; const int *site2pat; double *out; unsigned long long seed; int nsites, nboot; };
void launch_sh(const ShReq *reqs, int n, hipStream_t s);
#ifdef __HIPCC__
__device__ __forceinline__ unsigned long long mix64(unsigned long long z) {
    z ^= z >> 30; z *= 0xBF58476D1CE4E5B9ull; z ^= z >> 27; z *= 0x94D049BB133111EBull; z ^= z >> 31;
    return z;
}
#endif

struct RellReq {
    const double *X;
    const double *L;
    const int *ndraws;
    const double *scale;
    unsigned long long *bp;
    unsigned long long *kh, *sh;
    double *Y;
    unsigned long long base;
    unsigned B;
    int N, T, tpad, K, k1;
};
struct RellWReq : RellReq {
    const double *isig;
    unsigned long long *wkh, *wsh;
};
constexpr int rell_lds_slots(int tpad) { return (tpad / 2) | 1; }
constexpr size_t rell_lds_bytes(int N, int tpad) { return (size_t)N * rell_lds_slots(tpad) * 16; }
void launch_rell_pack(const double *const *src , const int *site2pat, double *X, double *L,
                      int N, int T, int tpad, hipStream_t s);
hipError_t launch_rell(const RellReq &r, bool lds, hipStream_t s);
bool rell_lds_fits(int N, int tpad, int device);
void launch_rell_pairsd(const double *X, double *isig, int N, int T, int tpad, hipStream_t s);
hipError_t launch_rell_weighted(const RellWReq &r, bool lds, hipStream_t s);
bool rell_weighted_lds_fits(int N, int tpad, int device);

void launch_pmat(const ModelDev *model, const PmatReq *reqs, double *frags, int n, hipStream_t s, bool per_request = false,
                 hipEvent_t start = nullptr, hipEvent_t stop = nullptr);
void launch_model_build(const ModelReq *reqs, int n, hipStream_t s, hipEvent_t start = nullptr, hipEvent_t stop = nullptr);
void launch_eigfrags(const ModelDev *model, double *frags2, hipStream_t s);
void launch_eigfrags_n(const ModelDev *models, double *frags2, int n, hipStream_t s);
void launch_oplist(const NvOp *ops, const GeneRun *runs, int nruns, int max_mpad, bool any_pitch, bool chained, hipStream_t s, NewtonCtl *ctl = nullptr,
                   hipEvent_t start = nullptr, hipEvent_t stop = nullptr);
void launch_reduce(const ReduceReq *reqs, int n, hipStream_t s, hipEvent_t start = nullptr, hipEvent_t stop = nullptr);
void launch_newton(const ModelDev *model, const NewtonReq *reqs, const int *tickets, int nreg, int nstream, NewtonCtl *ctl, hipStream_t s);
void launch_newton_seq(const ModelDev *model, const NewtonReq *reqs, const int *req_list, int nreg, int nstream, NewtonCtl *ctl, hipStream_t s);

}
```

pepr_amd/csrc/kernels.hip:

```cpp
#include "kernels.h"
#include <hip/hip_ext.h>

#include <algorithm>
#include <cstdlib>

namespace pml {

#define TWO_P256 1.15792089237316195423570985008687907853269984665640564039457584007913129639936e77
#define TWO_M256 8.63616855509444462538635186280017219262570580443837358382049248904e-78
#define LOG_2_256 177.445678223345993274051579105116

__device__ __forceinline__ double mfma4(double a, double b, double c) {
#ifdef ABL_NO_MFMA
    return __builtin_fma(a, b, c);
#endif
    return __builtin_amdgcn_mfma_f64_4x4x4f64(a, b, c, 0, 0, 0);
}

__device__ __forceinline__ unsigned code_mask(unsigned code) {
    return code < 20u ? (1u << code) : (code == 20u ? 0xCu : (code == 21u ? 0x60u : 0xFFFFFu));
}

template <int CTRL>
__device__ __forceinline__ double quad_swap(double v) {
    int lo = __double2loint(v), hi = __double2hiint(v);
    lo = __builtin_amdgcn_update_dpp(0, lo, CTRL, 0xF, 0xF, true);
    hi = __builtin_amdgcn_update_dpp(0, hi, CTRL, 0xF, 0xF, true);
    return __hiloint2double(hi, lo);
}
__device__ __forceinline__ double quad_sum(double v) { v += quad_swap<0xB1>(v); v += quad_swap<0x4E>(v); return v; }

__device__ __forceinline__ void frag_decode(int idx, int &c, int &row, int &col) {
    const int e = idx & 15, f = idx >> 4;
    c = f / 25;
    const int st = (f % 25) / 5, kk = f % 5;
    row = 4 * st + (e & 3); col = 4 * kk + (e >> 2);
}

constexpr int PMAT_THREADS = 256;
template <bool PER_REQ>
__global__ __launch_bounds__(PMAT_THREADS, 2) void k_pmat(const ModelDev *__restrict__ md0,
                                                          const PmatReq *__restrict__ reqs,
                                                          double *__restrict__ frags, int n) {
    __shared__ double sE[PMAT_THREADS / 64][NCAT * NS];
    const int lane = threadIdx.x & 63;
    const int wv = __builtin_amdgcn_readfirstlane(threadIdx.x >> 6);
    const int i4 = lane & 3, k4 = lane >> 4, cb = (lane >> 2) & 3;
    double Au[5][5], Bu[5][5];
    double lam0, lam1, pi_row[5];
    const int cat0 = lane / NS, cat1 = (64 + (lane & 15)) / NS;
    auto load_model = [&](const ModelDev *__restrict__ md) {
#pragma unroll
        for (int a = 0; a < 5; ++a)
#pragma unroll
            for (int b = 0; b < 5; ++b) {
                Au[a][b] = md->U[(4 * a + i4) * NS + 4 * b + k4];
                Bu[a][b] = md->Uinv[(4 * a + k4) * NS + 4 * b + i4];
            }
        lam0 = md->eval[lane % NS]; lam1 = md->eval[(64 + (lane & 15)) % NS];
#pragma unroll
        for (int a = 0; a < 5; ++a) pi_row[a] = md->pi[4 * a + k4];
    };
    if (!PER_REQ) load_model(md0);
    const int nwaves = gridDim.x * (PMAT_THREADS / 64);
    for (int rq = blockIdx.x * (PMAT_THREADS / 64) + wv; rq < n; rq += nwaves) {
        const PmatReq &req = reqs[rq];
        if (PER_REQ) load_model(req.md);
        const double tlen = req.tp ? *req.tp : req.t;
        const int kind = req.kind;
        double *sEw = sE[wv];
        sEw[lane] = exp(lam0 * (tlen * req.rates[cat0]));
        if (lane < 16) sEw[64 + lane] = exp(lam1 * (tlen * req.rates[cat1]));
        __builtin_amdgcn_fence(__ATOMIC_RELEASE, "wavefront");
        __builtin_amdgcn_wave_barrier();
        double ek[5];
#pragma unroll
        for (int kk = 0; kk < 5; ++kk) ek[kk] = sEw[cb * NS + 4 * kk + k4];
        __builtin_amdgcn_wave_barrier();
        double *out = frags + (size_t)rq * FRAG_STRIDE;
        double T[5][5];
#pragma unroll
        for (int st = 0; st < 5; ++st) {
            double a[5];
#pragma unroll
            for (int kk = 0; kk < 5; ++kk) a[kk] = Au[st][kk] * ek[kk];
#pragma unroll
            for (int nt = 0; nt < 5; ++nt) {
                double d = 0.0;
#pragma unroll
                for (int kk = 0; kk < 5; ++kk) d = mfma4(a[kk], Bu[kk][nt], d);
                T[st][nt] = d < 0.0 ? 0.0 : d;
            }
        }
        if (kind != PM_TIPTABLE) {
#pragma unroll
            for (int st = 0; st < 5; ++st) {
                const double scale = kind == PM_FRAGS_PI ? pi_row[st] : 1.0;
#pragma unroll
                for (int nt = 0; nt < 5; ++nt)
                    out[((cb * 25 + st * 5 + nt) << 4) + (i4 << 2) + k4] = T[st][nt] * scale;
            }
        } else {
            auto put = [&](int code, double v0, double v1, double v2, double v3, double v4) {
                typedef double dv2 __attribute__((ext_vector_type(2)));
                dv2 *rec = reinterpret_cast<dv2 *>(out + ((cb * NCODES + code) * 4 + k4) * TIPTAB_KK);
                rec[0] = (dv2){v0, v1}; rec[1] = (dv2){v2, v3}; rec[2] = (dv2){v4, 0.0};
            };
#pragma unroll
            for (int nt = 0; nt < 5; ++nt) put(4 * nt + i4, T[0][nt], T[1][nt], T[2][nt], T[3][nt], T[4][nt]);
            double bz[5], zq[5], any[5];
#pragma unroll
            for (int st = 0; st < 5; ++st) {
                bz[st] = T[st][0] + quad_swap<0xB1>(T[st][0]);
                zq[st] = T[st][1] + quad_swap<0xD8>(T[st][1]);
                any[st] = quad_sum(T[st][0] + T[st][1] + T[st][2] + T[st][3] + T[st][4]);
            }
            if (i4 == 2) put(20, bz[0], bz[1], bz[2], bz[3], bz[4]);
            if (i4 == 1) put(21, zq[0], zq[1], zq[2], zq[3], zq[4]);
            if (i4 == 0) put(22, any[0], any[1], any[2], any[3], any[4]);
        }
    }
}

__global__ __launch_bounds__(256) void k_eigfrags(const ModelDev *__restrict__ models,
                                                  double *__restrict__ frags2_all) {
    const ModelDev *__restrict__ md = models + blockIdx.x;
    double *__restrict__ frags2 = frags2_all + (size_t)blockIdx.x * 2 * PFRAG;
    for (int idx = threadIdx.x; idx < PFRAG; idx += 256) {
        int c, i, s;
        frag_decode(idx, c, i, s);
        frags2[idx] = md->pi[s] * md->U[s * NS + i];
        frags2[PFRAG + idx] = md->Uinv[i * NS + s];
    }
}

constexpr int MODEL_THREADS = 64;
constexpr int MODEL_MAX_SWEEPS = 40;
__global__ __launch_bounds__(MODEL_THREADS) void k_model(const ModelReq *__restrict__ reqs) {
    __shared__ double sB[NS * NS], sV[NS * NS], sPi[NS], sRt[NS], sRow[NS];
    __shared__ int sOrd[NS];
    const ModelReq &rq = reqs[blockIdx.x];
    const int lane = threadIdx.x;
    for (int e = lane; e < NS * (NS - 1) / 2; e += MODEL_THREADS) {
        int i = 1;
        while (i * (i + 1) / 2 <= e) ++i;
        const int j = e - i * (i - 1) / 2;
        const double v = e == rq.patch ? rq.patch_val : rq.exch[e];
        sV[i * NS + j] = v; sV[j * NS + i] = v;
    }
    if (lane < NS) { sPi[lane] = rq.pi[lane]; sV[lane * (NS + 1)] = 0.0; }
    __syncthreads();
    double sum = 0.0;
    for (int i = 0; i < NS; ++i) sum += sPi[i];
    __syncthreads();
    if (lane < NS) { const double p = sPi[lane] / sum; sPi[lane] = p; sRt[lane] = sqrt(p); }
    __syncthreads();
    if (lane < NS) {
        double row = 0.0;
        for (int j = 0; j < NS; ++j) if (j != lane) row += sV[lane * NS + j] * sPi[j];
        sRow[lane] = row;
    }
    __syncthreads();
    double mu = 0.0;
    for (int i = 0; i < NS; ++i) mu += sPi[i] * sRow[i];
    for (int e = lane; e < NS * NS; e += MODEL_THREADS) {
        const int i = e / NS, j = e % NS;
        const double qij = (i == j ? -sRow[i] : sV[e] * sPi[j]) / mu, qji = (i == j ? -sRow[i] : sV[e] * sPi[i]) / mu;
        const double bij = sRt[i] * qij / sRt[j], bji = sRt[j] * qji / sRt[i];
        sB[e] = i == j ? bij : 0.5 * (bij + bji);
    }
    __syncthreads();
    for (int e = lane; e < NS * NS; e += MODEL_THREADS) sV[e] = (e / NS == e % NS) ? 1.0 : 0.0;
    __syncthreads();
    const int k = lane % 10, i0 = lane / 10;
    for (int sweep = 0; sweep < MODEL_MAX_SWEEPS; ++sweep) {
        if (lane < NS) {
            double o = 0.0;
            for (int j = lane + 1; j < NS; ++j) o += sB[lane * NS + j] * sB[lane * NS + j];
            sRow[lane] = o;
        }
        __syncthreads();
        double off = 0.0;
        for (int i = 0; i < NS; ++i) off += sRow[i];
        if (off < 1e-40) break;
        for (int r = 0; r < NS - 1; ++r) {
            const int a = k == 0 ? NS - 1 : (r + k) % (NS - 1), b = k == 0 ? r : (r + NS - 1 - k) % (NS - 1);
            const int p = a < b ? a : b, q = a < b ? b : a;
            const double app = sB[p * (NS + 1)], aqq = sB[q * (NS + 1)], apq = sB[p * NS + q];
            double c = 1.0, s = 0.0;
            if (fabs(apq) >= 1e-300) {
                const double theta = (aqq - app) / (2.0 * apq);
                const double t = (theta >= 0.0 ? 1.0 : -1.0) / (fabs(theta) + sqrt(theta * theta + 1.0));
                c = 1.0 / sqrt(t * t + 1.0); s = t * c;
            }
            __syncthreads();
            if (lane < 50) {
#pragma unroll
                for (int it = 0; it < 4; ++it) {
                    const int i = i0 + 5 * it;
                    const double x = sB[i * NS + p], y = sB[i * NS + q];
                    sB[i * NS + p] = c * x - s * y; sB[i * NS + q] = s * x + c * y;
                    const double vx = sV[i * NS + p], vy = sV[i * NS + q];
                    sV[i * NS + p] = c * vx - s * vy; sV[i * NS + q] = s * vx + c * vy;
// ... 413 lines not shown
                    if (n1) v.y *= TWO_P256;
                    *ptr = v;
                }
            }
        }
        if (q == 0) { sc.x += n0 ? 1 : 0; sc.y += n1 ? 1 : 0; if (keep) *reinterpret_cast<GLOBAL_AS ivec2 *>((gptr)out_scl + 4 * p) = sc; }
        if (CHAIN) xsc = sc;
    } else if (mode == MODE_SUMTABLE || mode == MODE_EVALUATE_CAT) {
        if (fusedN) xsc = sc;
        else if (q == 0) *reinterpret_cast<GLOBAL_AS ivec2 *>((gptr)out_scl + 4 * p) = sc;
    } else {
        site0 += __shfl_xor(site0, 16); site0 += __shfl_xor(site0, 32);
        site1 += __shfl_xor(site1, 16); site1 += __shfl_xor(site1, 32);
        if (q == 0) {
            const double l0 = log(site0 * 0.25) - sc.x * LOG_2_256;
            const double l1 = log(site1 * 0.25) - sc.y * LOG_2_256;
            *reinterpret_cast<GLOBAL_AS dvec2 *>(O + 8 * p) = (dvec2){l0, l1};
        }
    }
}

constexpr int PAT_PER_WG = 4 * PAT_PER_WAVE;
constexpr int TIPTAB = NCODES * NS;

#ifndef PML_CHAIN_WAVES
#define PML_CHAIN_WAVES 2
#endif
__device__ __forceinline__ void dma_chunk(const double *set, double *lds_set, int k, int lane) {
    const GLOBAL_AS char *src = (const GLOBAL_AS char *)set + k * 4096 + lane * 16;
    __attribute__((address_space(3))) char *dst = (__attribute__((address_space(3))) char *)lds_set + k * 4096;
    if (k < 3) {
        __builtin_amdgcn_global_load_lds((const GLOBAL_AS void *)src, (__attribute__((address_space(3))) void *)dst, 16, 0, 0);
        __builtin_amdgcn_global_load_lds((const GLOBAL_AS void *)src, (__attribute__((address_space(3))) void *)dst, 16, 1024, 0);
        __builtin_amdgcn_global_load_lds((const GLOBAL_AS void *)src, (__attribute__((address_space(3))) void *)dst, 16, 2048, 0);
        __builtin_amdgcn_global_load_lds((const GLOBAL_AS void *)src, (__attribute__((address_space(3))) void *)dst, 16, 3072, 0);
    } else if (lane < 32) __builtin_amdgcn_global_load_lds((const GLOBAL_AS void *)src, (__attribute__((address_space(3))) void *)dst, 16, 0, 0);
}
__device__ __forceinline__ void stage_frags_dma3(const NvOp &op, double *dst, int lane, int wave) {
    const int wv = __builtin_amdgcn_readfirstlane(wave);
    const double *pl = op.pl, *pr = op.pr;
    const int lk = op.flags & 3, rk = (op.flags >> 2) & 3;
    const double *inner = (lk == SK_PITCH) ? op.l.f : (rk == SK_PITCH) ? op.r.f : nullptr;
    dma_chunk(pl ? pl : pr, dst, wv, lane);
    dma_chunk(pr ? pr : pl, dst + PFRAG, (wv + 1) & 3, lane);
    if (inner != nullptr) dma_chunk(inner, dst + 2 * PFRAG, (wv + 2) & 3, lane);
}

__device__ __forceinline__ void dma_rows4(const double *src, double *lds, int row, int lane) {
    const GLOBAL_AS char *s = (const GLOBAL_AS char *)src + row * 1024 + lane * 16;
    __attribute__((address_space(3))) char *d = (__attribute__((address_space(3))) char *)lds + row * 1024;
    __builtin_amdgcn_global_load_lds((const GLOBAL_AS void *)s, (__attribute__((address_space(3))) void *)d, 16, 0, 0);
    __builtin_amdgcn_global_load_lds((const GLOBAL_AS void *)s, (__attribute__((address_space(3))) void *)d, 16, 1024, 0);
    __builtin_amdgcn_global_load_lds((const GLOBAL_AS void *)s, (__attribute__((address_space(3))) void *)d, 16, 2048, 0);
    __builtin_amdgcn_global_load_lds((const GLOBAL_AS void *)s, (__attribute__((address_space(3))) void *)d, 16, 3072, 0);
}
__device__ __forceinline__ void dma_row(const double *src, double *lds, int row, int lane, int nlanes) {
    const GLOBAL_AS char *s = (const GLOBAL_AS char *)src + row * 1024 + lane * 16;
    __attribute__((address_space(3))) char *d = (__attribute__((address_space(3))) char *)lds + row * 1024;
    if (lane < nlanes) __builtin_amdgcn_global_load_lds((const GLOBAL_AS void *)s, (__attribute__((address_space(3))) void *)d, 16, 0, 0);
}
static_assert(PFRAG * 8 == 12 * 1024 + 32 * 16 && TIPTAB_DOUBLES * 8 == 17 * 1024 + 16 * 16, "rows of a fragment set and of a tip table");
__device__ __forceinline__ void stage_frags_wide(const NvOp &op, double *dst, int lane, int wave) {
    const int wv = __builtin_amdgcn_readfirstlane(wave);
    const double *pl = op.pl, *pr = op.pr;
    const int lk = op.flags & 3, rk = (op.flags >> 2) & 3;
    const double *inner = (lk == SK_PITCH) ? op.l.f : (rk == SK_PITCH) ? op.r.f : nullptr;
    const double *L = pl ? pl : pr, *R = pr ? pr : pl;
    if (wv < 3) dma_rows4(L, dst, 4 * wv, lane);
    else if (wv < 6) dma_rows4(R, dst + PFRAG, 4 * (wv - 3), lane);
    else dma_row(wv == 6 ? L : R, wv == 6 ? dst : dst + PFRAG, 12, lane, 32);
    if (inner != nullptr) {
        if (wv >= 5) dma_rows4(inner, dst + 2 * PFRAG, 4 * (wv - 5), lane);
        else if (wv == 4) dma_row(inner, dst + 2 * PFRAG, 12, lane, 32);
    }
    if (lk >= SK_CHERRY || rk >= SK_CHERRY) {
        const double *ta = lk >= SK_CHERRY ? op.l.t0 : op.r.t0, *tb = lk >= SK_CHERRY ? op.l.t1 : op.r.t1;
        double *da = dst + 3 * PFRAG, *db = da + TIPTAB_DOUBLES;
        if (wv < 4) dma_rows4(ta, da, 4 * wv, lane); else dma_rows4(tb, db, 4 * (wv - 4), lane);
        if (wv < 2) dma_row(ta, da, 16 + wv, lane, wv == 0 ? 64 : 16);
        else if (wv < 4) dma_row(tb, db, 14 + wv, lane, wv == 2 ? 64 : 16);
    }
}

struct FusedShared {
    double exl[NCAT * NS][2];
    double red[3];
    double fb[3][PAT_PER_WAVE * 4];
    double ss[PAT_PER_WAVE * 4];
    double bc[4];
};
static_assert(sizeof(FusedShared) <= PFRAG * sizeof(double), "fused Newton scratch fits one fragment region");
__device__ __forceinline__ void newton_fused(const NvOp &op, double *scratch, const Operand (&X)[4], const ivec2 xsc,
                                             bool active, int blk, NewtonCtl *ctl, long long timeout_ticks) {
    const NewtonReq &r = *reinterpret_cast<const NewtonReq *>(op.aux);
    FusedShared &sh = *reinterpret_cast<FusedShared *>(scratch);
    const int tid = threadIdx.x, lane = tid & 63, wave = tid >> 6, q = lane >> 4, pl = wave * PAT_PER_WAVE + 2 * (lane & 15);
    const int mpad = r.mpad, S = newton_split(mpad);
    const ModelDev *__restrict__ md = r.md;
    u64 *gran = reinterpret_cast<u64 *>(r.sync);
    __syncthreads();
    if (q == 0) { sh.ss[pl] = active ? (double)xsc.x : 0.0; sh.ss[pl + 1] = active ? (double)xsc.y : 0.0; }
    if (tid == 0) sh.bc[3] = 0.0;
    double sw = 0.0;
    if (wave < 2) { const int pf = blk * (PAT_PER_WAVE * 4) + wave * 64 + lane; if (pf < mpad) sw = r.weight[pf]; }
    int nevals = 0;
    auto eval_at = [&](double t, double &L, double &d1, double &d2) -> bool {
        if (tid < NCAT * NS) {
            const double lr = md->eval[tid % NS] * r.rates[tid / NS];
            sh.exl[tid][0] = exp(lr * t); sh.exl[tid][1] = lr;
        }
        __syncthreads();
        double fa = 0.0, fa1 = 0.0, fa2 = 0.0, fb = 0.0, fb1 = 0.0, fb2 = 0.0;
#pragma unroll
        for (int c = 0; c < NCAT; ++c)
#pragma unroll
            for (int st = 0; st < 5; ++st) {
                const int row = c * NS + 4 * st + q;
                const double e = sh.exl[row][0], lr = sh.exl[row][1];
                newton_term(X[c].v[st].x, e, lr, fa, fa1, fa2);
                newton_term(X[c].v[st].y, e, lr, fb, fb1, fb2);
            }
        fa += __shfl_xor(fa, 16); fa += __shfl_xor(fa, 32); fa1 += __shfl_xor(fa1, 16); fa1 += __shfl_xor(fa1, 32); fa2 += __shfl_xor(fa2, 16); fa2 += __shfl_xor(fa2, 32);
        fb += __shfl_xor(fb, 16); fb += __shfl_xor(fb, 32); fb1 += __shfl_xor(fb1, 16); fb1 += __shfl_xor(fb1, 32); fb2 += __shfl_xor(fb2, 16); fb2 += __shfl_xor(fb2, 32);
        if (q == 0) {
            sh.fb[0][pl] = fa; sh.fb[1][pl] = fa1; sh.fb[2][pl] = fa2;
            sh.fb[0][pl + 1] = fb; sh.fb[1][pl + 1] = fb1; sh.fb[2][pl + 1] = fb2;
        }
        __syncthreads();
        double tot[3] = {0.0, 0.0, 0.0};
        if (wave < 2) {
            double a0 = 0.0, a1 = 0.0, a2 = 0.0;
            if (sw != 0.0) {
                const int j = wave * 64 + lane;
                newton_finish(sh.fb[0][j], sh.fb[1][j], sh.fb[2][j], sw, sh.ss[j], a0, a1, a2);
            }
            tot[0] = wave_sum(a0); tot[1] = wave_sum(a1); tot[2] = wave_sum(a2);
            if (wave == 0 && lane == 0) { sh.red[0] = tot[0]; sh.red[1] = tot[1]; sh.red[2] = tot[2]; }
        }
        __syncthreads();
        if (wave == 1) {
#pragma unroll
            for (int i = 0; i < 3; ++i) tot[i] = sh.red[i] + __shfl(tot[i], 0);
            bool bad = false;
            if (S > 1) bad = newton_exchange(gran, S, blk, nevals, r.tag_base, tot, ctl, timeout_ticks);
            if (lane == 0) { sh.bc[0] = tot[0]; sh.bc[1] = tot[1]; sh.bc[2] = tot[2]; if (bad) sh.bc[3] = 1.0; }
        }
        __syncthreads();
        ++nevals;
        L = uni(sh.bc[0]); d1 = uni(sh.bc[1]); d2 = uni(sh.bc[2]);
        return sh.bc[3] == 0.0;
    };
    double t, L, d1, d2;
    const bool ok = newton_drive(r.t0, r.max_iter, r.tol, eval_at, t, L, d1, d2);
    if (tid == 64 && blk == 0) {
        atomicAdd(&ctl->n_requests, 1ull); atomicAdd(&ctl->n_evals, (unsigned long long)nevals);
        if (!ok) { t = r.t0; L = __builtin_nan(""); }
        r.out[0] = t; r.out[1] = L; r.out[2] = d1; r.out[3] = d2;
        if (r.t_dev0) { *r.t_dev0 = t; *r.t_dev1 = t; }
    }
}

#ifdef PML_OPTIME
__device__ unsigned long long g_optime[256][2];
}
extern "C" void pml_abl_optime(unsigned long long *out, int reset) {
    (void)hipDeviceSynchronize();
    (void)hipMemcpyFromSymbol(out, HIP_SYMBOL(pml::g_optime), sizeof(unsigned long long) * 512);
    if (reset) { static unsigned long long z[512]; (void)hipMemcpyToSymbol(HIP_SYMBOL(pml::g_optime), z, sizeof z); }
}
namespace pml {
#endif
template <bool CHAIN, bool DBUF, bool FUSE, int WAVES>
__device__ __forceinline__ void oplist_body(
        const NvOp *__restrict__ ops, const GeneRun *__restrict__ runs, int nruns, int blocks_per_gene, int any_pitch,
        NewtonCtl *ctl, long long timeout_ticks) {
    static_assert(CHAIN || !DBUF, "LDS-DMA staging exists for the chained kernels only");
    static_assert(!FUSE || (CHAIN && DBUF), "the fused-Newton kernel is the scoring kernel plus the Newton code");
    static_assert(WAVES == 4 || (WAVES == 8 && CHAIN && DBUF && !FUSE), "eight waves: the scoring kernel only");
    constexpr bool WIDE = WAVES == 8;
    constexpr int WG_PAT = WAVES * PAT_PER_WAVE;
#ifdef PML_OPTIME
    const long long t_life0 = clock64();
#endif
    constexpr int PARITY_STRIDE = 3 * PFRAG + (WIDE ? 2 * TIPTAB_DOUBLES : 0);
    Operand X[4]; ivec2 xsc = {0, 0};
#pragma unroll
    for (int c = 0; c < 4; ++c)
#pragma unroll
        for (int k = 0; k < 5; ++k) X[c].v[k] = (dvec2){0.0, 0.0};
    extern __shared__ double sP[];
    const int nfrag_doubles = DBUF ? 2 * PARITY_STRIDE : (2 + (any_pitch ? 1 : 0)) * PFRAG;
    unsigned char *sT = reinterpret_cast<unsigned char *>(sP + nfrag_doubles);
    const int tid = threadIdx.x, lane = tid & 63, wave = tid >> 6;
    const bool one_part = blocks_per_gene < 0;
    if (one_part) blocks_per_gene = -blocks_per_gene;
    const int xcd = one_part ? 0 : (blockIdx.x & 7);
    int slot = one_part ? (int)blockIdx.x : (int)(blockIdx.x >> 3);
    const bool ticketed = FUSE && ctl != nullptr;
    if (ticketed) {
        __shared__ int s_slot;
        if (tid == 0) s_slot = __hip_atomic_fetch_add(&ctl->oticket[xcd], 1, __ATOMIC_RELAXED, __HIP_MEMORY_SCOPE_AGENT);
        __syncthreads();
        slot = s_slot;
    }
    auto leave = [&]() {
        if (!ticketed) return;
        __syncthreads();
        if (tid == 0) {
            const int d = __hip_atomic_fetch_add(&ctl->odone, 1, __ATOMIC_RELAXED, __HIP_MEMORY_SCOPE_AGENT);
            if (d == (int)gridDim.x - 1) {
#pragma unroll
                for (int k = 0; k < 8; ++k) __hip_atomic_store(&ctl->oticket[k], 0, __ATOMIC_RELAXED, __HIP_MEMORY_SCOPE_AGENT);
                __hip_atomic_store(&ctl->odone, 0, __ATOMIC_RELAXED, __HIP_MEMORY_SCOPE_AGENT);
            }
        }
    };
    const int gi = one_part ? slot / blocks_per_gene : xcd + 8 * (slot / blocks_per_gene), blk = slot % blocks_per_gene;
    if (gi >= nruns) { leave(); return; }
    const GeneRun run = runs[gi];
    if (run.op_begin >= run.op_end) { leave(); return; }
    const int mpad = ops[run.op_begin].mpad;
    if (blk * WG_PAT >= mpad) { leave(); return; }
    const int p = (blk * WAVES + wave) * PAT_PER_WAVE + 2 * (lane & 15);
    const bool active = (blk * WAVES + wave) * PAT_PER_WAVE < mpad;

#ifdef PML_OPTIME
    const long long t_start1 = clock64();
#endif
    for (int i = tid; i < TIPTAB; i += 64 * WAVES) sT[i] = (unsigned char)((code_mask(i / NS) >> (i % NS)) & 1u);
    auto stage = [&](const NvOp &o, double *dst) { if (WIDE) stage_frags_wide(o, dst, lane, wave); else stage_frags_dma3(o, dst, lane, wave); };
    if (DBUF) stage(ops[run.op_begin], sP);
    __syncthreads();
#ifdef PML_OPTIME
    const long long t_start2 = clock64();
    long long t_newton = 0, t_bar = 0, t_ops = 0;
#endif
    for (int oi = run.op_begin; oi < run.op_end; ++oi) {
        const NvOp &op = ops[oi];
        const double *buf = sP;
        if (DBUF) {
            const int par = (oi - run.op_begin) & 1;
            buf = sP + par * PARITY_STRIDE;
            if (oi + 1 < run.op_end) stage(ops[oi + 1], sP + (par ^ 1) * PARITY_STRIDE);
        } else {
            if (oi > run.op_begin) __syncthreads();
            const double2 *gl = reinterpret_cast<const double2 *>(op.pl);
            const double2 *gr = reinterpret_cast<const double2 *>(op.pr);
            double2 *s2 = reinterpret_cast<double2 *>(sP);
            for (int i = tid; i < PFRAG / 2; i += 256) {
                if (op.mode < MODE_EVALUATE && op.pl) s2[i] = gl[i];
                if (op.pr) s2[PFRAG / 2 + i] = gr[i];
            }
            if (any_pitch) {
                const int lk = op.flags & 3, rk = (op.flags >> 2) & 3;
                const double2 *il = reinterpret_cast<const double2 *>(op.l.f), *ir = reinterpret_cast<const double2 *>(op.r.f);
                for (int i = tid; i < PFRAG / 2; i += 256) {
                    if (lk == SK_PITCH) s2[PFRAG + i] = il[i];
                    else if (rk == SK_PITCH) s2[PFRAG + i] = ir[i];
                }
            }
            __syncthreads();
        }
#ifdef PML_OPTIME
        const long long t_op0 = clock64();
#endif
#ifndef ABL_NO_OP
        if (active) chunk_op<CHAIN, FUSE, WIDE>(op, buf, sT, p, lane, X, xsc);
#endif
#ifdef PML_OPTIME
        if (lane == 0 && active) {
            const int k = (op.flags & 15) | ((op.mode & 3) << 4) | ((op.flags & (OPF_CHAIN_L | OPF_CHAIN_R)) ? 64 : 0) | ((op.flags & OPF_NO_STORE) ? 128 : 0);
            atomicAdd(&g_optime[k][0], (unsigned long long)(clock64() - t_op0)); atomicAdd(&g_optime[k][1], 1ull);
        }
        t_ops += clock64() - t_op0;
        const long long t_n0 = clock64();
#endif
        if (FUSE && (op.flags & OPF_FUSED_NEWTON) != 0) {
            if (__hip_atomic_load(&ctl->abort, __ATOMIC_RELAXED, __HIP_MEMORY_SCOPE_AGENT) != 0) {
                const NewtonReq &r = *reinterpret_cast<const NewtonReq *>(op.aux);
                if (tid == 0 && blk == 0) { r.out[0] = r.t0; r.out[1] = __builtin_nan(""); r.out[2] = 0.0; r.out[3] = 0.0; }
            } else newton_fused(op, const_cast<double *>(buf), X, xsc, active, blk, ctl, timeout_ticks);
        }
#ifdef PML_OPTIME
        const long long t_b0 = clock64(); t_newton += t_b0 - t_n0;
#endif
#ifndef ABL_NO_BARRIER
        if (DBUF) __syncthreads();
#endif
#ifdef PML_OPTIME
        t_bar += clock64() - t_b0;
#endif
    }
#ifdef PML_OPTIME
    if (lane == 0 && active) {
        const int b = FUSE ? 230 : 238;
        const long long t_end = clock64();
        atomicAdd(&g_optime[b][0], (unsigned long long)(t_end - t_life0)); atomicAdd(&g_optime[b][1], 1ull);
        atomicAdd(&g_optime[b + 1][0], (unsigned long long)(t_start1 - t_life0)); atomicAdd(&g_optime[b + 2][0], (unsigned long long)(t_start2 - t_start1));
        atomicAdd(&g_optime[b + 3][0], (unsigned long long)t_ops); atomicAdd(&g_optime[b + 4][0], (unsigned long long)t_newton); atomicAdd(&g_optime[b + 5][0], (unsigned long long)t_bar);
    }
#endif
    leave();
}
template <bool CHAIN, bool DBUF, bool FUSE>
__global__ __launch_bounds__(256, CHAIN ? PML_CHAIN_WAVES : 4) void k_oplist(
        const NvOp *__restrict__ ops, const GeneRun *__restrict__ runs, int nruns, int blocks_per_gene, int any_pitch,
        NewtonCtl *ctl, long long timeout_ticks) {
    oplist_body<CHAIN, DBUF, FUSE, 4>(ops, runs, nruns, blocks_per_gene, any_pitch, ctl, timeout_ticks);
}
__global__ __launch_bounds__(512, PML_CHAIN_WAVES) void k_oplist_wide(
        const NvOp *__restrict__ ops, const GeneRun *__restrict__ runs, int nruns, int blocks_per_gene, int any_pitch,
        NewtonCtl *ctl, long long timeout_ticks) {
    oplist_body<true, true, false, 8>(ops, runs, nruns, blocks_per_gene, any_pitch, ctl, timeout_ticks);
}

constexpr auto k_oplist_plain = k_oplist<false, false, false>;
constexpr auto k_oplist_chain1 = k_oplist<true, false, false>;
constexpr auto k_oplist_score = k_oplist<true, true, false>;
constexpr auto k_oplist_newton = k_oplist<true, true, true>;

template <int N, int WAVES>
__device__ __forceinline__ void block_sum(double (&v)[N], double (*red)[WAVES]) {
    const int lane = threadIdx.x & 63, wave = threadIdx.x >> 6;
#pragma unroll
    for (int i = 0; i < N; ++i) { const double s = wave_sum(v[i]); if (lane == 0) red[i][wave] = s; }
    __syncthreads();
#pragma unroll
    for (int i = 0; i < N; ++i) {
        double s = red[i][0];
#pragma unroll
        for (int w = 1; w < WAVES; ++w) s += red[i][w];
        v[i] = s;
    }
    __syncthreads();
}

__global__ __launch_bounds__(256) void k_reduce(const ReduceReq *__restrict__ reqs) {
    __shared__ double red[1][4];
    const ReduceReq r = reqs[blockIdx.x];
    double acc[1] = {0.0};
    for (int p = threadIdx.x; p < r.mpad; p += 256) {
        const double w = r.weight[p];
        if (w != 0.0) acc[0] += w * r.patlnl[p];
    }
    block_sum<1, 4>(acc, red);
    if (threadIdx.x == 0) *r.out = acc[0];
}

constexpr int NEWTON_THREADS = 512;
constexpr int NEWTON_WAVES = NEWTON_THREADS / 64;
constexpr int NEWTON_SLICE = NEWTON_WAVES * 16;
constexpr int NEWTON_ROWS = CLV_ROWS / 4;
static_assert(NEWTON_SLICE == NEWTON_SLICE_PAT, "kernels.h newton_split / newton_slice describe this kernel's slices");

struct NewtonShared {
    double exl[NCAT * NS][2];
    double red[3][NEWTON_WAVES];
    double fb[3][NEWTON_SLICE];
    double xs[2][NEWTON_ROWS][64];
    double part[3][NEWTON_MAX_SPLIT];
    double bc[4];
    int ticket;
};

// ... 208 lines not shown
    }
}

__global__ __launch_bounds__(256) void k_sh(const ShReq *__restrict__ reqs) {
    __shared__ double red[3][4];
    const ShReq r = reqs[blockIdx.x];
    const int tid = threadIdx.x;
    double orig[3] = {0.0, 0.0, 0.0};
    for (int j = tid; j < r.nsites; j += 256) { const int p = r.site2pat[j]; orig[0] += r.l0[p]; orig[1] += r.l1[p]; orig[2] += r.l2[p]; }
    block_sum<3, 4>(orig, red);
    const double delta = orig[0] - fmax(orig[1], orig[2]);
    double cnt[1] = {0.0};
    if (delta > 0.0) {
        const unsigned long long base = (r.seed + 1ull) * 0x9E3779B97F4A7C15ull, ns = (unsigned long long)r.nsites;
        for (int b = tid; b < r.nboot; b += 256) {
            double s0 = 0.0, s1 = 0.0, s2 = 0.0;
            const unsigned long long k0 = base + (unsigned long long)b * ns;
            for (int j = 0; j < r.nsites; ++j) {
                const int p = r.site2pat[(int)(mix64(k0 + (unsigned long long)j) % ns)];
                s0 += r.l0[p]; s1 += r.l1[p]; s2 += r.l2[p];
            }
            s0 -= orig[0]; s1 -= orig[1]; s2 -= orig[2];
            const double best = fmax(s0, fmax(s1, s2));
            const double second = (best == s0) ? fmax(s1, s2) : (best == s1 ? fmax(s0, s2) : fmax(s0, s1));
            if (best - second < delta) cnt[0] += 1.0;
        }
    }
    __shared__ double red1[1][4];
    block_sum<1, 4>(cnt, red1);
    if (tid == 0) *r.out = (r.nboot > 0) ? cnt[0] / (double)r.nboot : 0.0;
}

__global__ __launch_bounds__(256) void k_g20(const G20Req *__restrict__ reqs) {
    __shared__ double red[1][4];
    __shared__ double w[G20_RATES];
    const G20Req &r = reqs[blockIdx.x];
    if (threadIdx.x < G20_RATES) w[threadIdx.x] = r.w[threadIdx.x];
    __syncthreads();
    const size_t M = (size_t)r.mpad;
    double acc[1] = {0.0};
    for (int p = threadIdx.x; p < r.mpad; p += 256) {
        const double wt = r.weight[p];
        double l = 0.0;
        if (wt != 0.0) {
            int m = r.cnt[p];
#pragma unroll
            for (int j = 1; j < G20_RATES / 4; ++j) m = min(m, r.cnt[(size_t)j * M + p]);
            double sum = 0.0;
#pragma unroll
            for (int j = 0; j < G20_RATES / 4; ++j) {
                const int d = r.cnt[(size_t)j * M + p] - m;
                const double f = ldexp(1.0, -256 * d);
#pragma unroll
                for (int c = 0; c < 4; ++c) sum += w[4 * j + c] * r.table[(size_t)(4 * j + c) * M + p] * f;
            }
            l = log(sum) - m * LOG_2_256;
            acc[0] += wt * l;
        }
        if (r.patlnl) r.patlnl[p] = l;
    }
    block_sum<1, 4>(acc, red);
    if (threadIdx.x == 0) *r.out = acc[0];
}

void launch_g20(const G20Req *reqs, int n, hipStream_t s) {
    if (n <= 0) return;
    hipLaunchKernelGGL(k_g20, dim3((unsigned)n), dim3(256), 0, s, reqs);
}
void launch_sh(const ShReq *reqs, int n, hipStream_t s) {
    if (n <= 0) return;
    hipLaunchKernelGGL(k_sh, dim3((unsigned)n), dim3(256), 0, s, reqs);
}
void launch_gather(const GatherSeg *segs, int nsegs, int max_npat, hipStream_t s) {
    if (nsegs <= 0 || max_npat <= 0) return;
    hipLaunchKernelGGL(k_gather, dim3((unsigned)nsegs, (unsigned)((max_npat + 255) / 256)), dim3(256), 0, s, segs);
}
void launch_pmat(const ModelDev *model, const PmatReq *reqs, double *frags, int n, hipStream_t s, bool per_request, hipEvent_t start, hipEvent_t stop) {
    if (n <= 0) return;
    const int per_block = PMAT_THREADS / 64;
    const int blocks = std::min((n + per_block - 1) / per_block, 512);
    if (per_request) hipExtLaunchKernelGGL(k_pmat<true>, dim3(blocks), dim3(PMAT_THREADS), 0, s, start, stop, 0, model, reqs, frags, n);
    else hipExtLaunchKernelGGL(k_pmat<false>, dim3(blocks), dim3(PMAT_THREADS), 0, s, start, stop, 0, model, reqs, frags, n);
}
void launch_eigfrags(const ModelDev *model, double *frags2, hipStream_t s) {
    hipLaunchKernelGGL(k_eigfrags, dim3(1), dim3(256), 0, s, model, frags2);
}
void launch_eigfrags_n(const ModelDev *models, double *frags2, int n, hipStream_t s) {
    if (n > 0) hipLaunchKernelGGL(k_eigfrags, dim3((unsigned)n), dim3(256), 0, s, models, frags2);
}
void launch_model_build(const ModelReq *reqs, int n, hipStream_t s, hipEvent_t start, hipEvent_t stop) {
    if (n > 0) hipExtLaunchKernelGGL(k_model, dim3((unsigned)n), dim3(MODEL_THREADS), 0, s, start, stop, 0, reqs);
}
static long long newton_timeout_ticks();
static void launch_oplist_one(const NvOp *ops, const GeneRun *runs, int nruns, int bpg, bool one_part, bool any_pitch, bool chained, hipStream_t s, NewtonCtl *ctl,
                              hipEvent_t start = nullptr, hipEvent_t stop = nullptr);
void launch_oplist(const NvOp *ops, const GeneRun *runs, int nruns, int max_mpad, bool any_pitch, bool chained, hipStream_t s, NewtonCtl *ctl,
                   hipEvent_t start, hipEvent_t stop) {
    if (nruns <= 0) return;
    const int bpg = (max_mpad + PAT_PER_WG - 1) / PAT_PER_WG;
    if (!ctl) { launch_oplist_one(ops, runs, nruns, bpg, false, any_pitch, chained, s, nullptr, start, stop); return; }
    launch_oplist_one(ops, runs, nruns, bpg, bpg > 32, any_pitch, true, s, ctl);
}
static void launch_oplist_one(const NvOp *ops, const GeneRun *runs, int nruns, int bpg_in, bool one_part, bool any_pitch, bool chained, hipStream_t s, NewtonCtl *ctl,
                              hipEvent_t start, hipEvent_t stop) {
    const long long to = newton_timeout_ticks();
    const int bpg = one_part ? -bpg_in : bpg_in;
    const dim3 grid((unsigned)(one_part ? nruns * bpg_in : ((nruns + 7) / 8) * 8 * bpg_in)), block(256);
    const int ap = any_pitch ? 1 : 0;
    const size_t lds_single = (size_t)(2 + ap) * PFRAG * sizeof(double) + 512;
    const size_t lds_double = (size_t)6 * PFRAG * sizeof(double) + 512;
    const size_t lds_wide = (size_t)2 * (3 * PFRAG + 2 * TIPTAB_DOUBLES) * sizeof(double) + 512;
    if (!chained) {
        hipExtLaunchKernelGGL(k_oplist_plain, grid, block, lds_single, s, start, stop, 0, ops, runs, nruns, bpg, ap, ctl, to);
        return;
    }
    static const hipError_t big = [&] {
        const hipError_t a = hipFuncSetAttribute(reinterpret_cast<const void *>(k_oplist_score), hipFuncAttributeMaxDynamicSharedMemorySize, (int)lds_double);
        const hipError_t b = hipFuncSetAttribute(reinterpret_cast<const void *>(k_oplist_newton), hipFuncAttributeMaxDynamicSharedMemorySize, (int)lds_double);
        return a != hipSuccess ? a : b;
    }();
    static const int variant = std::getenv("PML_CHAIN_VARIANT") ? std::atoi(std::getenv("PML_CHAIN_VARIANT")) : 0;
    static const bool want_chain1 = variant == 9;
    static const hipError_t big_wide = hipFuncSetAttribute(reinterpret_cast<const void *>(k_oplist_wide), hipFuncAttributeMaxDynamicSharedMemorySize, (int)lds_wide);
    if (!ctl && !one_part && variant == 0 && big_wide == hipSuccess && bpg_in > 1) {
        const int bpg_wide = (bpg_in + 1) / 2;
        hipExtLaunchKernelGGL(k_oplist_wide, dim3((unsigned)(((nruns + 7) / 8) * 8 * bpg_wide)), dim3(512), lds_wide, s, start, stop, 0, ops, runs, nruns, bpg_wide, ap, ctl, to);
        return;
    }
    if (ctl) hipExtLaunchKernelGGL(k_oplist_newton, grid, block, lds_double, s, start, stop, 0, ops, runs, nruns, bpg, ap, ctl, to);
    else if (want_chain1 || big != hipSuccess) hipExtLaunchKernelGGL(k_oplist_chain1, grid, block, lds_single, s, start, stop, 0, ops, runs, nruns, bpg, ap, ctl, to);
    else hipExtLaunchKernelGGL(k_oplist_score, grid, block, lds_double, s, start, stop, 0, ops, runs, nruns, bpg, ap, ctl, to);
}
void launch_reduce(const ReduceReq *reqs, int n, hipStream_t s, hipEvent_t start, hipEvent_t stop) {
    if (n <= 0) return;
    hipExtLaunchKernelGGL(k_reduce, dim3(n), dim3(256), 0, s, start, stop, 0, reqs);
}
static long long newton_timeout_ticks() {
    static const long long v = [] { const char *e = std::getenv("PML_NEWTON_TIMEOUT_US"); return e ? std::atoll(e) * 100LL : 2000000LL * 100LL; }();
    return v;
}
void launch_newton(const ModelDev *model, const NewtonReq *reqs, const int *tickets, int nreg, int nstream, NewtonCtl *ctl, hipStream_t s) {
    const long long to = newton_timeout_ticks();
    if (nreg > 0) hipLaunchKernelGGL((k_newton<true, false>), dim3((unsigned)nreg), dim3(NEWTON_THREADS), 0, s, model, reqs, tickets, ctl, to);
    if (nstream > 0) hipLaunchKernelGGL((k_newton<false, false>), dim3((unsigned)nstream), dim3(NEWTON_THREADS), 0, s, model, reqs, tickets + nreg, ctl, to);
}
void launch_newton_seq(const ModelDev *model, const NewtonReq *reqs, const int *req_list, int nreg, int nstream, NewtonCtl *ctl, hipStream_t s) {
    if (nreg > 0) hipLaunchKernelGGL((k_newton<true, true>), dim3((unsigned)nreg), dim3(NEWTON_THREADS), 0, s, model, reqs, req_list, ctl, 0LL);
    if (nstream > 0) hipLaunchKernelGGL((k_newton<false, true>), dim3((unsigned)nstream), dim3(NEWTON_THREADS), 0, s, model, reqs, req_list + nreg, ctl, 0LL);
}

}
```

Baseline: 190.1.

## Cache per-branch transition matrices in persistent slots and emit them from Newton tails

Adds a per-gene arena of transition-matrix slots tagged by branch length, model epoch and rates, so unchanged branches reuse matrices across launches instead of re-running k_pmat for them. The fused Newton branch optimiser now also writes the matrices for the optimised branch directly into these slots after convergence, which removes the follow-up k_pmat requests in chained smoothing passes. The cost is extra device memory per gene, host-side tag bookkeeping, and invalidation logic that could serve stale matrices if any model change fails to bump the epoch. The fused kernel now also zeroes operand registers after Newton.

```diff
diff --git a/__graft_entry__.py b/__graft_entry__.py
--- a/__graft_entry__.py
+++ b/__graft_entry__.py
@@ -20,6 +20,9 @@
     subprocess.check_call(["g++", "-O1", "-std=c++17", "-fPIC", "-shared", "-Wall", "-Werror", "-D__HIP_PLATFORM_AMD__", "-I" + os.path.join(rocm, "include"),
                            os.path.join(d, "kh.cpp"), "-L" + os.path.join(ROOT, "pepr_amd"), "-lpeprml", "-L" + os.path.join(rocm, "lib"), "-lamdhip64",
                            "-Wl,-rpath,$ORIGIN/../../pepr_amd", "-Wl,-rpath," + os.path.join(rocm, "lib"), "-o", os.path.join(d, "libkh.so")])
+    subprocess.check_call(["g++", "-O1", "-std=c++17", "-fPIC", "-shared", "-Wall", "-Werror", "-D__HIP_PLATFORM_AMD__", "-I" + os.path.join(rocm, "include"),
+                           os.path.join(d, "kh_fused.cpp"), "-L" + os.path.join(ROOT, "pepr_amd"), "-lpeprml", "-L" + os.path.join(rocm, "lib"), "-lamdhip64",
+                           "-Wl,-rpath,$ORIGIN/../../pepr_amd", "-Wl,-rpath," + os.path.join(rocm, "lib"), "-o", os.path.join(d, "libkh_fused.so")])
 
 
 def build():
diff --git a/pepr_amd/csrc/api.cpp b/pepr_amd/csrc/api.cpp
--- a/pepr_amd/csrc/api.cpp
+++ b/pepr_amd/csrc/api.cpp
@@ -204,7 +204,8 @@
 static size_t gene_bytes_bound(const pml_alignment &a, bool score_only) {
     const size_t mp = ((size_t)std::max(a.nsites, 1) + 31) / 32 * 32, nt = (size_t)std::max(a.ntax, 3);
     const size_t slots = (score_only ? nt - 2 : 3 * (nt - 2)) + NSCRATCH + MAXTAIL;
-    return slots * CLV_ROWS * ((mp + 127) / 128 * 128) * 8 + slots * mp * 4 + nt * mp + 64 * mp + (1 << 16);
+    const size_t mats = score_only ? 0 : (3 * nt + 8) * (size_t)FRAG_STRIDE * 8;
+    return slots * CLV_ROWS * ((mp + 127) / 128 * 128) * 8 + slots * mp * 4 + nt * mp + 64 * mp + (1 << 16) + mats;
 }
 
 static int oneshot_on(Ctx &c, int op, int n, const pml_alignment *alns, const char *const *newicks,
diff --git a/pepr_amd/csrc/engine.cpp b/pepr_amd/csrc/engine.cpp
--- a/pepr_amd/csrc/engine.cpp
+++ b/pepr_amd/csrc/engine.cpp
@@ -143,6 +143,7 @@
     for (int i = 0; i < NS; ++i) pi[i] /= sum;
 }
 int Batch::build_gene_models() {
+    ++model_epoch;
     const int n = (int)genes.size();
     if (int rc = alloc_gene_models()) return rc;
     std::vector<ModelDev> h(n);
@@ -172,6 +173,7 @@
     return 0;
 }
 int Batch::build_models(const std::vector<int> &gs, int patch, const double *vals) {
+    ++model_epoch;
     if (gs.empty()) return 0;
     static const bool host_arm = std::getenv("PML_MODEL_HOST") != nullptr;
     const int n = (int)genes.size(), m = (int)gs.size();
@@ -199,6 +201,7 @@
     return 0;
 }
 int Batch::set_matrix(int g, const double *exch, const double *pi) {
+    ++model_epoch;
     const int n = (int)genes.size();
     HIPCHK(hipSetDevice(ctx->device));
     if (!d_gmodel) {
@@ -357,6 +360,8 @@
         total += (size_t)MAXTAIL * clv_doubles(mp) * 8;
         total += (size_t)MAXTAIL * align_up((size_t)mp * 4, 256);
         total += (size_t)MAXTAIL * align_up((size_t)mp * 8, 256);
+        G.mat_cap = score_only ? 0 : 3 * nt + 8;
+        total += (size_t)G.mat_cap * FRAG_STRIDE * 8;
     }
     arena_bytes = total;
     const double t_alloc0 = now_ms();
@@ -382,6 +387,8 @@
         for (int k = 0; k < MAXTAIL; ++k) { G.d_sumtab[k] = (double *)p; p += clv_doubles(mp) * 8; }
         for (int k = 0; k < MAXTAIL; ++k) { G.d_sumscl[k] = (int *)p; p += align_up((size_t)mp * 4, 256); }
         for (int k = 0; k < MAXTAIL; ++k) { G.d_patlnl[k] = (double *)p; p += align_up((size_t)mp * 8, 256); }
+        G.d_mats = (double *)p; p += (size_t)G.mat_cap * FRAG_STRIDE * 8;
+        G.mat_tag.assign((size_t)G.mat_cap, Gene::MatTag()); G.mat_of.clear(); G.mat_next = 0; G.mat_reset = false;
         if (!G.aln.codes.empty()) {
             HIPCHK(hipMemcpyAsync(G.d_codes, G.aln.codes.data(), (size_t)nt * mp, hipMemcpyHostToDevice, ctx->stream));
             HIPCHK(hipMemcpyAsync(G.d_weight, G.aln.weight.data(), (size_t)mp * 8, hipMemcpyHostToDevice, ctx->stream));
@@ -417,6 +424,8 @@
             NewtonCtl h[2];
             if (hipMemcpy(h, d_nctl, sizeof h, hipMemcpyDeviceToHost) == hipSuccess && h[0].n_requests)
                 fprintf(stderr, "[pml] branch Newton: %llu requests, %.2f evaluations each\n", h[0].n_requests, (double)h[0].n_evals / (double)h[0].n_requests);
+            fprintf(stderr, "[pml] matrices of chained passes: %ld smoothing steps, %ld k_pmat launches with %ld requests; persistent slots: %ld found built, %ld built by Newton tails\n",
+                    cnt_smooth, cnt_pmat_launches, cnt_pmat_reqs, cnt_mats_hit, cnt_mats_emitted);
         }
         hipFree(d_nctl); d_nctl = nullptr;
     }
@@ -806,7 +815,9 @@
         ctx->tic_stream = st;
         if (L.nreq) {
             ctx->tic(K_PMAT, (double)L.nreq * PFRAG * 8);
-            launch_pmat(md, (const PmatReq *)(ds + L.o_req), frags_buf, (int)L.nreq, st, d_gmodel != nullptr);
+            if (chain) { ++cnt_pmat_launches; cnt_pmat_reqs += (long)L.nreq; }
+            if (L.to_slots) launch_pmat_to(md, (const PmatReq *)(ds + L.o_req), (double *const *)(ds + L.o_out), (int)L.nreq, st, d_gmodel != nullptr);
+            else launch_pmat(md, (const PmatReq *)(ds + L.o_req), frags_buf, (int)L.nreq, st, d_gmodel != nullptr);
             ctx->toc(); PML_SER();
         }
         if (L.nruns) {
@@ -827,7 +838,10 @@
             ctx->toc(); PML_SER();
         }
         ctx->tic_stream = nullptr;
-        if (hipError_t e = hipGetLastError(); e != hipSuccess) return ctx->fail(-5, std::string("kernel launch: ") + hipGetErrorString(e));
+        if (hipError_t e = hipGetLastError(); e != hipSuccess) {
+            for (auto &G : genes) G.mats_invalidate();
+            return ctx->fail(-5, std::string("kernel launch: ") + hipGetErrorString(e));
+        }
     }
 #undef PML_SER
     flush_quota = std::min<size_t>(flush_quota * 2, 8);
@@ -841,6 +855,9 @@
     const size_t nops = ops.size(), ntail = tails.size();
     size_t neval = 0, nnewton = 0;
     for (auto &t : tails) { if (t.mode == MODE_EVALUATE) neval++; else if (t.mode != MODE_EVALUATE_CAT) nnewton++; }
+    static const bool mats_env = !(std::getenv("PML_PMAT_EMIT") && std::atoi(std::getenv("PML_PMAT_EMIT")) == 0);
+    const bool use_mats = mats_env && !record_plan && !lanes_active && lane == 0;
+    if (!use_mats) prefetch_mats = false;
     size_t nreq_max = 10 * nops + 9 * ntail;
     {
         std::vector<char> seen(genes.size(), 0);
@@ -849,7 +866,7 @@
                               if (o.out_kind != SIDE_MSG) loose += (o.bv[0] < 0) + (o.bv[1] < 0); }
         for (auto &t : tails) { if (!seen[t.gene]) { seen[t.gene] = 1; keyed += 5 * (size_t)genes[t.gene].aln.ntax; }
                                 if (t.mode >= MODE_EVALUATE && t.bv < 0) loose += 1; }
-        nreq_max = std::min(nreq_max, keyed + loose);
+        nreq_max = prefetch_mats ? keyed + loose : std::min(nreq_max, keyed + loose);
     }
     bool any_pitch = false, any_chain = false;
     if (int rc = ensure_frags(std::max(nreq_max, (size_t)1))) return rc;
@@ -887,7 +904,9 @@
     size_t ntick_max = 0;
     for (auto &t : tails) if (t.mode == MODE_SUMTABLE) ntick_max += (size_t)newton_split(genes[t.gene].aln.mpad);
     const size_t o_tick = align_up(o_newt + nnewton * sizeof(NewtonReq), 256);
-    const size_t bytes = align_up(o_tick + ntick_max * sizeof(int), 256);
+    const size_t o_out = align_up(o_tick + ntick_max * sizeof(int), 256);
+    const size_t o_emit = align_up(o_out + (use_mats ? nreq_max : 0) * sizeof(double *), 256);
+    const size_t bytes = align_up(o_emit + (use_mats ? nnewton : 0) * sizeof(NewtonEmit), 256);
     if (chain && chain_off + bytes > h_cap) { if (int rc = chain_sync()) return rc; }
     if (int rc = ensure_stage(bytes)) return rc;
     const size_t base = chain ? chain_off : 0;
@@ -899,6 +918,8 @@
     ReduceReq *hred = (ReduceReq *)(hs + o_red);
     NewtonReq *hnewt = (NewtonReq *)(hs + o_newt);
     int *htick = (int *)(hs + o_tick);
+    double **hout = (double **)(hs + o_out);
+    NewtonEmit *hemit = (NewtonEmit *)(hs + o_emit);
     if (nnewton) ++newton_launch_seq;
     const unsigned tag_base = (newton_launch_seq & 0x3FFFFFu) << 10;
     static const bool fuse_env = std::getenv("PML_NO_FUSE") == nullptr && !(std::getenv("PML_CHAIN") && std::atoi(std::getenv("PML_CHAIN")) == 0);
@@ -909,6 +930,7 @@
 
     size_t nout = 0, nruns = 0, ie = 0, in = 0, ireq = 0, iop = 0;
     last_src.clear();
+    struct MatsGuard { Batch *b; bool issued = false; ~MatsGuard() { if (!issued) for (auto &G : b->genes) G.mats_invalidate(); } } mats_guard{this};
     int max_mpad = 0, newton_maxm = 0;
     double algo_bytes = 0, algo_flops = 0;
     bool req_ok = req_off.size() == genes.size() + 1;
@@ -919,6 +941,18 @@
         req_stamp.assign(req_off.back(), 0); req_ptr.assign(req_off.back(), nullptr); req_launch = 0;
         val_bucket.assign(genes.size() * 3, {}); val_stamp.assign(genes.size() * 3, 0);
     }
+    if (use_mats) for (auto &G : genes) {
+        const size_t nd = (size_t)3 * G.tree.nnodes();
+        if (G.mat_of.size() != 3 * nd) { G.mat_of.assign(3 * nd, -1); G.mat_reset = true; }
+        if (G.mat_reset) G.mats_clear();
+        if (G.pend_seq.size() != nd) G.pend_seq.assign(nd, 0);
+    }
+    auto mat_slot = [&](Gene &G, int kind, size_t bkey) -> int {
+        if (G.mat_cap == 0) return -1;
+        int &pi = G.mat_of[(size_t)kind * 3 * G.tree.nnodes() + bkey];
+        if (pi < 0) { if (G.mat_next >= G.mat_cap) { G.mat_reset = true; return -1; } pi = G.mat_next++; }
+        return pi;
+    };
     if (++req_launch == 0) {
         std::fill(req_stamp.begin(), req_stamp.end(), 0u); std::fill(val_stamp.begin(), val_stamp.end(), 0u); req_launch = 1;
     }
@@ -926,12 +960,26 @@
     auto add_req = [&](size_t g, double t, int kind, int v, int q) -> const double * {
         uint64_t tbits = 0; size_t key = 0;
         std::vector<std::pair<uint64_t, const double *>> *bucket = nullptr;
+        double *slot = nullptr;
         if (!record_plan) {
             if (v >= 0) {
-                const Tree &T = genes[g].tree;
+                Gene &G = genes[g];
+                const Tree &T = G.tree;
                 const int w = T.nbr[v][q], a = v * 3 + q, b = w * 3 + T.slot(w, v);
                 key = req_off[g] + (size_t)kind * 3 * T.nnodes() + (size_t)std::min(a, b);
                 if (req_stamp[key] == req_launch) return req_ptr[key];
+                const int pi = use_mats ? mat_slot(G, kind, (size_t)std::min(a, b)) : -1;
+                if (pi >= 0) {
+                    const bool pending = chain && G.len_pending[(size_t)v * 3 + q];
+                    Gene::MatTag &tg = G.mat_tag[pi];
+                    std::memcpy(&tbits, &t, 8);
+                    slot = G.d_mats + (size_t)pi * FRAG_STRIDE;
+                    const bool hit = tg.state != 0 && tg.model_epoch == model_epoch && std::memcmp(tg.rates, G.rates, sizeof tg.rates) == 0 &&
+                                     (pending ? tg.state == 2 && tg.seq == G.pend_seq[(size_t)v * 3 + q] : tg.state == 1 && tg.tbits == tbits);
+                    if (hit) { ++cnt_mats_hit; req_stamp[key] = req_launch; req_ptr[key] = slot; return slot; }
+                    tg.state = pending ? 2 : 1; tg.tbits = tbits; tg.seq = pending ? G.pend_seq[(size_t)v * 3 + q] : 0;
+                    tg.model_epoch = model_epoch; std::memcpy(tg.rates, G.rates, sizeof tg.rates);
+                }
             } else {
                 std::memcpy(&tbits, &t, 8);
                 const size_t bi = g * 3 + (size_t)kind;
@@ -946,7 +994,9 @@
         r.tp = (chain && v >= 0 && genes[g].len_pending[(size_t)v * 3 + q]) ? genes[g].d_len + (size_t)v * 3 + q : nullptr;
         r.md = d_gmodel ? d_gmodel + g : nullptr;
         last_src.push_back({(int)g, v, q, kind});
-        const double *out = frags_buf + (ireq++) * FRAG_STRIDE;
+        double *out = slot ? slot : frags_buf + ireq * FRAG_STRIDE;
+        if (use_mats) hout[ireq] = out;
+        ++ireq;
         if (!record_plan) { if (v >= 0) { req_stamp[key] = req_launch; req_ptr[key] = out; } else bucket->push_back({tbits, out}); }
         return out;
     };
@@ -994,6 +1044,23 @@
         return 0;
     };
 
+    if (prefetch_mats && use_mats && chain) {
+        for (auto &t : tails) {
+            if (t.mode != MODE_SUMTABLE || t.bv < 0 || !t.t_dev0) continue;
+            Gene &G = genes[t.gene];
+            const Tree &T = G.tree;
+            const int nt = G.aln.ntax, skip = t.bv * 3 + t.bq;
+            for (int v = 0; v < T.nnodes(); ++v) for (int q = 0; q < 3; ++q) {
+                const int w = T.nbr[v][q];
+                if (w < 0) continue;
+                const int a = v * 3 + q, b = w * 3 + T.slot(w, v);
+                if (a > b || a == skip || b == skip) continue;
+                add_req((size_t)t.gene, T.len[v][q], PM_FRAGS, v, q);
+                if (v < nt || w < nt) add_req((size_t)t.gene, T.len[v][q], PM_TIPTABLE, v, q);
+            }
+        }
+    }
+    prefetch_mats = false;
     std::vector<std::vector<int>> &tails_of = run_tails_of;
     if (tails_of.size() < nkeys) tails_of.resize(nkeys);
     for (auto &v : tails_of) v.clear();
@@ -1051,9 +1118,31 @@
                 d.out = stab; d.out_scl = sscl;
                 NewtonReq &nr = hnewt[in];
                 nr.md = model_of((int)g); nr.tag_base = tag_base; nr.pad0 = 0;
-                if (fuse_ok && !t.patlnl_dev && newton_reg_form(mp)) {
+                const bool fuse_this = fuse_ok && !t.patlnl_dev && newton_reg_form(mp);
+                if (fuse_this) {
                     d.flags |= OPF_FUSED_NEWTON; d.aux = (const NewtonReq *)(ds + o_newt) + in;
                     fused_req[in] = 1; any_fused = true; any_chain = true;
+                }
+                if (use_mats && chain && t.t_dev0 && t.bv >= 0) {
+                    const Tree &T = G.tree;
+                    const int v = t.bv, q = t.bq, w = T.nbr[v][q], a = v * 3 + q, b = w * 3 + T.slot(w, v);
+                    const unsigned seq = ++pend_counter;
+                    G.pend_seq[a] = G.pend_seq[b] = seq;
+                    if (fuse_this && t.after < 0 && nparts[g] == 1 && tails_of[key].size() == 1) {
+                        NewtonEmit &E = hemit[in];
+                        std::memset(&E, 0, sizeof E);
+                        const int kinds[2] = {PM_FRAGS, PM_TIPTABLE};
+                        for (int ki = 0; ki < ((v < G.aln.ntax || w < G.aln.ntax) ? 2 : 1); ++ki) {
+                            const int kind = kinds[ki];
+                            if (req_stamp[req_off[g] + (size_t)kind * 3 * T.nnodes() + (size_t)std::min(a, b)] == req_launch) continue;
+                            const int pi = mat_slot(G, kind, (size_t)std::min(a, b));
+                            if (pi < 0) continue;
+                            Gene::MatTag &tg = G.mat_tag[pi];
+                            tg.state = 2; tg.tbits = 0; tg.seq = seq; tg.model_epoch = model_epoch; std::memcpy(tg.rates, G.rates, sizeof tg.rates);
+                            E.out[E.n] = G.d_mats + (size_t)pi * FRAG_STRIDE; E.kind[E.n] = kind; ++E.n;
+                        }
+                        if (E.n) { d.pad = (int)((o_emit + in * sizeof(NewtonEmit)) - (o_newt + in * sizeof(NewtonReq))); cnt_mats_emitted += E.n; }
+                    }
                 }
                 last_nv = -1; last_nv_op = -1;
                 tail_req[&t - tails.data()] = (int)in;
@@ -1121,6 +1210,7 @@
     }
 
     if (req_overflow) return ctx->fail(-5, "internal: transition-matrix request bound exceeded");
+    mats_guard.issued = true;
     int nt_reg = 0, nt_stream = 0;
     const bool seq_launch = nnewton > 0 && newton_safe_mode();
     {
@@ -1140,7 +1230,7 @@
     for (size_t i = 0; i < ntail; ++i) if (tails[i].mode == MODE_SUMTABLE && !fused_req[tail_req[i]]) newton_bytes += (double)genes[tails[i].gene].aln.npat * 640;
     Deferred L;
     L.base = base; L.bytes = bytes; L.o_req = o_req; L.o_ops = o_ops; L.o_runs = o_runs; L.o_red = o_red; L.o_newt = o_newt;
-    L.o_tick = o_tick; L.nt_reg = nt_reg; L.nt_stream = nt_stream; L.seq = seq_launch; L.fused = any_fused;
+    L.o_tick = o_tick; L.o_out = o_out; L.to_slots = use_mats; L.nt_reg = nt_reg; L.nt_stream = nt_stream; L.seq = seq_launch; L.fused = any_fused;
     L.nreq = ireq; L.nruns = nruns; L.neval = neval; L.nnewton = nnewton; L.max_mpad = max_mpad; L.newton_maxm = newton_maxm;
     L.any_pitch = any_pitch; L.any_chain = any_chain; L.algo_bytes = algo_bytes; L.algo_flops = algo_flops; L.newton_bytes = newton_bytes; L.lane = lane; L.stagger = record_stagger;
     record_stagger = false;
@@ -1394,12 +1484,14 @@
                 if (chain) {
                     t.result_dev = d_chain + 4 * done.size();
                     t.t_dev0 = G.d_len + (size_t)v * 3 + G.tree.slot(v, w); t.t_dev1 = G.d_len + (size_t)w * 3 + G.tree.slot(w, v);
+                    t.bv = v; t.bq = G.tree.slot(v, w);
                 }
                 done.push_back({g, v, w, t.t0, done.size()});
                 tails.push_back(t);
             }
             if (tails.empty()) continue;
             lane = ln;
+            prefetch_mats = chain && step == 0;
             if (two_lanes && step == 0) {
                 if (!ev_stagger) hipEventCreateWithFlags(&ev_stagger, hipEventDisableTiming);
                 if (ln == 0) record_stagger = true;
@@ -1438,7 +1530,7 @@
             if (attempt == 1 || safe_now) return ctx->fail(-5, "k_newton: non-finite branch likelihood (also from the no-exchange form)");
             newton_gave_up(); ctx->newton_reissued += (long long)done.size();
             if (int rc = clear_abort()) return rc;
-            for (int g = 0; g < n; ++g) if (active[g]) { std::fill(genes[g].len_pending.begin(), genes[g].len_pending.end(), 0); invalidate_all(g); }
+            for (int g = 0; g < n; ++g) if (active[g]) { std::fill(genes[g].len_pending.begin(), genes[g].len_pending.end(), 0); invalidate_all(g); genes[g].mats_invalidate(); }
             safe_now = true;
             continue;
         }
@@ -1448,6 +1540,16 @@
             det_record(det_id, G, 'S', d.v, d.w, d.old, nl, h_chain[4 * d.idx + 1]);
             maxdelta[d.gene] = std::max(maxdelta[d.gene], dl);
             G.tree.set_len(d.v, d.w, nl);
+            if (!G.mat_of.empty() && !G.pend_seq.empty()) {
+                const int a = d.v * 3 + G.tree.slot(d.v, d.w), b = d.w * 3 + G.tree.slot(d.w, d.v);
+                const double cur = G.tree.len[d.v][G.tree.slot(d.v, d.w)];
+                for (int kind = 0; kind < 3; ++kind) {
+                    const int pi = G.mat_of[(size_t)kind * 3 * G.tree.nnodes() + (size_t)std::min(a, b)];
+                    if (pi < 0 || G.mat_tag[pi].state != 2) continue;
+                    Gene::MatTag &tg = G.mat_tag[pi];
+                    if (tg.seq == G.pend_seq[a] && cur == nl) { tg.state = 1; std::memcpy(&tg.tbits, &nl, 8); } else tg.state = 0;
+                }
+            }
             if (dl > thr) { std::swap(G.dirty, next[d.gene]); G.mark_node(d.v); G.mark_node(d.w); std::swap(G.dirty, next[d.gene]); }
         }
         for (auto &G : genes) std::fill(G.len_pending.begin(), G.len_pending.end(), 0);
diff --git a/pepr_amd/csrc/engine.hpp b/pepr_amd/csrc/engine.hpp
--- a/pepr_amd/csrc/engine.hpp
+++ b/pepr_amd/csrc/engine.hpp
@@ -81,6 +81,13 @@
     std::vector<uint8_t> dirty;
     double *d_len = nullptr;
     std::vector<uint8_t> len_pending;
+    struct MatTag { uint64_t tbits = 0; double rates[NCAT] = {0, 0, 0, 0}; unsigned model_epoch = 0, seq = 0; uint8_t state = 0; };
+    double *d_mats = nullptr; int mat_cap = 0, mat_next = 0; bool mat_reset = false;
+    std::vector<int> mat_of;
+    std::vector<MatTag> mat_tag;
+    std::vector<unsigned> pend_seq;
+    void mats_clear() { std::fill(mat_of.begin(), mat_of.end(), -1); mat_next = 0; mat_reset = false; for (auto &t : mat_tag) t.state = 0; }
+    void mats_invalidate() { for (auto &t : mat_tag) t.state = 0; }
     void mark_node(int v) { for (int k = 0; k < 3; ++k) { const int w = tree.nbr[v][k]; if (w < 0) continue; dirty[v * 3 + k] = 1; dirty[w * 3 + tree.slot(w, v)] = 1; } }
     void mark_all() { dirty.assign((size_t)tree.nnodes() * 3, 1); }
     void mark_none() { dirty.assign((size_t)tree.nnodes() * 3, 0); }
@@ -178,9 +185,12 @@
     bool chain = false; size_t chain_off = 0;
     double *d_lenpool = nullptr;
     double *d_chain = nullptr, *h_chain = nullptr; size_t chain_cap = 0;
-    struct Deferred { size_t base, bytes, o_req, o_ops, o_runs, o_red, o_newt, o_tick, nreq, nruns, neval, nnewton; int nt_reg, nt_stream; bool seq, fused;
+    struct Deferred { size_t base, bytes, o_req, o_ops, o_runs, o_red, o_newt, o_tick, o_out, nreq, nruns, neval, nnewton; int nt_reg, nt_stream; bool seq, fused, to_slots;
                       int max_mpad, newton_maxm, lane; bool any_pitch, any_chain, stagger; double algo_bytes, newton_bytes, algo_flops; };
     std::vector<Deferred> deferred; size_t flush_quota = 1; bool lanes_active = false;
+    unsigned model_epoch = 1, pend_counter = 0;
+    bool prefetch_mats = false;
+    long cnt_pmat_launches = 0, cnt_pmat_reqs = 0, cnt_mats_emitted = 0, cnt_mats_hit = 0;
     int flush_deferred();
     int chain_begin(size_t nresults);
     int ensure_results(size_t nresults);
diff --git a/pepr_amd/csrc/kernels.h b/pepr_amd/csrc/kernels.h
--- a/pepr_amd/csrc/kernels.h
+++ b/pepr_amd/csrc/kernels.h
@@ -101,6 +101,11 @@
     int ticket0;
     int pad;
 };
+struct NewtonEmit {
+    double *out[3];
+    int kind[3];
+    int n;
+};
 constexpr int NEWTON_MAX_SPLIT = 64;
 constexpr int NEWTON_SLICE_PAT = 128;
 __host__ __device__ constexpr int newton_split(int mpad) { return (mpad + NEWTON_SLICE_PAT - 1) / NEWTON_SLICE_PAT < NEWTON_MAX_SPLIT ? ((mpad + NEWTON_SLICE_PAT - 1) / NEWTON_SLICE_PAT < 1 ? 1 : (mpad + NEWTON_SLICE_PAT - 1) / NEWTON_SLICE_PAT) : NEWTON_MAX_SPLIT; }
@@ -169,6 +174,7 @@
 
 void launch_pmat(const ModelDev *model, const PmatReq *reqs, double *frags, int n, hipStream_t s, bool per_request = false,
                  hipEvent_t start = nullptr, hipEvent_t stop = nullptr);
+void launch_pmat_to(const ModelDev *model, const PmatReq *reqs, double *const *outs, int n, hipStream_t s, bool per_request = false);
 void launch_model_build(const ModelReq *reqs, int n, hipStream_t s, hipEvent_t start = nullptr, hipEvent_t stop = nullptr);
 void launch_eigfrags(const ModelDev *model, double *frags2, hipStream_t s);
 void launch_eigfrags_n(const ModelDev *models, double *frags2, int n, hipStream_t s);
diff --git a/pepr_amd/csrc/kernels.hip b/pepr_amd/csrc/kernels.hip
--- a/pepr_amd/csrc/kernels.hip
+++ b/pepr_amd/csrc/kernels.hip
@@ -38,87 +38,93 @@
 }
 
 constexpr int PMAT_THREADS = 256;
-template <bool PER_REQ>
+struct PmatModel {
+    double Au[5][5], Bu[5][5];
+    double lam0, lam1, pi_row[5];
+};
+__device__ __forceinline__ void pmat_load_model(PmatModel &m, const ModelDev *__restrict__ md, int lane) {
+    const int i4 = lane & 3, k4 = lane >> 4;
+#pragma unroll
+    for (int a = 0; a < 5; ++a)
+#pragma unroll
+        for (int b = 0; b < 5; ++b) {
+            m.Au[a][b] = md->U[(4 * a + i4) * NS + 4 * b + k4];
+            m.Bu[a][b] = md->Uinv[(4 * a + k4) * NS + 4 * b + i4];
+        }
+    m.lam0 = md->eval[lane % NS]; m.lam1 = md->eval[(64 + (lane & 15)) % NS];
+#pragma unroll
+    for (int a = 0; a < 5; ++a) m.pi_row[a] = md->pi[4 * a + k4];
+}
+__device__ __forceinline__ void pmat_request(const PmatModel &m, double tlen, const double *__restrict__ rates, int kind,
+                                             double *__restrict__ out, double *sEw, int lane) {
+    const int i4 = lane & 3, k4 = lane >> 4, cb = (lane >> 2) & 3;
+    const int cat0 = lane / NS, cat1 = (64 + (lane & 15)) / NS;
+    sEw[lane] = exp(m.lam0 * (tlen * rates[cat0]));
+    if (lane < 16) sEw[64 + lane] = exp(m.lam1 * (tlen * rates[cat1]));
+    __builtin_amdgcn_fence(__ATOMIC_RELEASE, "wavefront");
+    __builtin_amdgcn_wave_barrier();
+    double ek[5];
+#pragma unroll
+    for (int kk = 0; kk < 5; ++kk) ek[kk] = sEw[cb * NS + 4 * kk + k4];
+    __builtin_amdgcn_wave_barrier();
+    double T[5][5];
+#pragma unroll
+    for (int st = 0; st < 5; ++st) {
+        double a[5];
+#pragma unroll
+        for (int kk = 0; kk < 5; ++kk) a[kk] = m.Au[st][kk] * ek[kk];
+#pragma unroll
+        for (int nt = 0; nt < 5; ++nt) {
+            double d = 0.0;
+#pragma unroll
+            for (int kk = 0; kk < 5; ++kk) d = mfma4(a[kk], m.Bu[kk][nt], d);
+            T[st][nt] = d < 0.0 ? 0.0 : d;
+        }
+    }
+    if (kind != PM_TIPTABLE) {
+#pragma unroll
+        for (int st = 0; st < 5; ++st) {
+            const double scale = kind == PM_FRAGS_PI ? m.pi_row[st] : 1.0;
+#pragma unroll
+            for (int nt = 0; nt < 5; ++nt)
+                out[((cb * 25 + st * 5 + nt) << 4) + (i4 << 2) + k4] = T[st][nt] * scale;
+        }
+    } else {
+        auto put = [&](int code, double v0, double v1, double v2, double v3, double v4) {
+            typedef double dv2 __attribute__((ext_vector_type(2)));
+            dv2 *rec = reinterpret_cast<dv2 *>(out + ((cb * NCODES + code) * 4 + k4) * TIPTAB_KK);
+            rec[0] = (dv2){v0, v1}; rec[1] = (dv2){v2, v3}; rec[2] = (dv2){v4, 0.0};
+        };
+#pragma unroll
+        for (int nt = 0; nt < 5; ++nt) put(4 * nt + i4, T[0][nt], T[1][nt], T[2][nt], T[3][nt], T[4][nt]);
+        double bz[5], zq[5], any[5];
+#pragma unroll
+        for (int st = 0; st < 5; ++st) {
+            bz[st] = T[st][0] + quad_swap<0xB1>(T[st][0]);
+            zq[st] = T[st][1] + quad_swap<0xD8>(T[st][1]);
+            any[st] = quad_sum(T[st][0] + T[st][1] + T[st][2] + T[st][3] + T[st][4]);
+        }
+        if (i4 == 2) put(20, bz[0], bz[1], bz[2], bz[3], bz[4]);
+        if (i4 == 1) put(21, zq[0], zq[1], zq[2], zq[3], zq[4]);
+        if (i4 == 0) put(22, any[0], any[1], any[2], any[3], any[4]);
+    }
+}
+template <bool PER_REQ, bool TO_SLOTS = false>
 __global__ __launch_bounds__(PMAT_THREADS, 2) void k_pmat(const ModelDev *__restrict__ md0,
                                                           const PmatReq *__restrict__ reqs,
                                                           double *__restrict__ frags, int n) {
     __shared__ double sE[PMAT_THREADS / 64][NCAT * NS];
     const int lane = threadIdx.x & 63;
     const int wv = __builtin_amdgcn_readfirstlane(threadIdx.x >> 6);
-    const int i4 = lane & 3, k4 = lane >> 4, cb = (lane >> 2) & 3;
-    double Au[5][5], Bu[5][5];
-    double lam0, lam1, pi_row[5];
-    const int cat0 = lane / NS, cat1 = (64 + (lane & 15)) / NS;
-    auto load_model = [&](const ModelDev *__restrict__ md) {
-#pragma unroll
-        for (int a = 0; a < 5; ++a)
-#pragma unroll
-            for (int b = 0; b < 5; ++b) {
-                Au[a][b] = md->U[(4 * a + i4) * NS + 4 * b + k4];
-                Bu[a][b] = md->Uinv[(4 * a + k4) * NS + 4 * b + i4];
-            }
-        lam0 = md->eval[lane % NS]; lam1 = md->eval[(64 + (lane & 15)) % NS];
-#pragma unroll
-        for (int a = 0; a < 5; ++a) pi_row[a] = md->pi[4 * a + k4];
-    };
-    if (!PER_REQ) load_model(md0);
+    PmatModel m;
+    if (!PER_REQ) pmat_load_model(m, md0, lane);
     const int nwaves = gridDim.x * (PMAT_THREADS / 64);
     for (int rq = blockIdx.x * (PMAT_THREADS / 64) + wv; rq < n; rq += nwaves) {
         const PmatReq &req = reqs[rq];
-        if (PER_REQ) load_model(req.md);
+        if (PER_REQ) pmat_load_model(m, req.md, lane);
         const double tlen = req.tp ? *req.tp : req.t;
-        const int kind = req.kind;
-        double *sEw = sE[wv];
-        sEw[lane] = exp(lam0 * (tlen * req.rates[cat0]));
-        if (lane < 16) sEw[64 + lane] = exp(lam1 * (tlen * req.rates[cat1]));
-        __builtin_amdgcn_fence(__ATOMIC_RELEASE, "wavefront");
-        __builtin_amdgcn_wave_barrier();
-        double ek[5];
-#pragma unroll
-        for (int kk = 0; kk < 5; ++kk) ek[kk] = sEw[cb * NS + 4 * kk + k4];
-        __builtin_amdgcn_wave_barrier();
-        double *out = frags + (size_t)rq * FRAG_STRIDE;
-        double T[5][5];
-#pragma unroll
-        for (int st = 0; st < 5; ++st) {
-            double a[5];
-#pragma unroll
-            for (int kk = 0; kk < 5; ++kk) a[kk] = Au[st][kk] * ek[kk];
-#pragma unroll
-            for (int nt = 0; nt < 5; ++nt) {
-                double d = 0.0;
-#pragma unroll
-                for (int kk = 0; kk < 5; ++kk) d = mfma4(a[kk], Bu[kk][nt], d);
-                T[st][nt] = d < 0.0 ? 0.0 : d;
-            }
-        }
-        if (kind != PM_TIPTABLE) {
-#pragma unroll
-            for (int st = 0; st < 5; ++st) {
-                const double scale = kind == PM_FRAGS_PI ? pi_row[st] : 1.0;
-#pragma unroll
-                for (int nt = 0; nt < 5; ++nt)
-                    out[((cb * 25 + st * 5 + nt) << 4) + (i4 << 2) + k4] = T[st][nt] * scale;
-            }
-        } else {
-            auto put = [&](int code, double v0, double v1, double v2, double v3, double v4) {
-                typedef double dv2 __attribute__((ext_vector_type(2)));
-                dv2 *rec = reinterpret_cast<dv2 *>(out + ((cb * NCODES + code) * 4 + k4) * TIPTAB_KK);
-                rec[0] = (dv2){v0, v1}; rec[1] = (dv2){v2, v3}; rec[2] = (dv2){v4, 0.0};
-            };
-#pragma unroll
-            for (int nt = 0; nt < 5; ++nt) put(4 * nt + i4, T[0][nt], T[1][nt], T[2][nt], T[3][nt], T[4][nt]);
-            double bz[5], zq[5], any[5];
-#pragma unroll
-            for (int st = 0; st < 5; ++st) {
-                bz[st] = T[st][0] + quad_swap<0xB1>(T[st][0]);
-                zq[st] = T[st][1] + quad_swap<0xD8>(T[st][1]);
-                any[st] = quad_sum(T[st][0] + T[st][1] + T[st][2] + T[st][3] + T[st][4]);
-            }
-            if (i4 == 2) put(20, bz[0], bz[1], bz[2], bz[3], bz[4]);
-            if (i4 == 1) put(21, zq[0], zq[1], zq[2], zq[3], zq[4]);
-            if (i4 == 0) put(22, any[0], any[1], any[2], any[3], any[4]);
-        }
+        double *out = TO_SLOTS ? reinterpret_cast<double *const *>(frags)[rq] : frags + (size_t)rq * FRAG_STRIDE;
+        pmat_request(m, tlen, req.rates, req.kind, out, sE[wv], lane);
     }
 }
 
@@ -698,6 +704,11 @@
     }
 }
 
+__device__ __noinline__ void newton_emit(const ModelDev *md, double t, const double *rates, int kind, double *out, double *sEw, int lane) {
+    PmatModel m;
+    pmat_load_model(m, md, lane);
+    pmat_request(m, t, rates, kind, out, sEw, lane);
+}
 struct FusedShared {
     double exl[NCAT * NS][2];
     double red[3];
@@ -705,7 +716,7 @@
     double ss[PAT_PER_WAVE * 4];
     double bc[4];
 };
-static_assert(sizeof(FusedShared) <= PFRAG * sizeof(double), "fused Newton scratch fits one fragment region");
+static_assert(sizeof(FusedShared) <= (PFRAG / 2) * sizeof(double) && PFRAG / 2 + 4 * NCAT * NS <= PFRAG, "fused Newton scratch and the emitting waves' rows fit one fragment region");
 __device__ __forceinline__ void newton_fused(const NvOp &op, double *scratch, const Operand (&X)[4], const ivec2 xsc,
                                              bool active, int blk, NewtonCtl *ctl, long long timeout_ticks) {
     const NewtonReq &r = *reinterpret_cast<const NewtonReq *>(op.aux);
@@ -774,6 +785,11 @@
         r.out[0] = t; r.out[1] = L; r.out[2] = d1; r.out[3] = d2;
         if (r.t_dev0) { *r.t_dev0 = t; *r.t_dev1 = t; }
     }
+    if (ok && blk == 0 && op.pad != 0) {
+        const NewtonEmit &em = *reinterpret_cast<const NewtonEmit *>(reinterpret_cast<const char *>(op.aux) + op.pad);
+        const int wv = __builtin_amdgcn_readfirstlane(wave);
+        if (wv < em.n) newton_emit(md, t, r.rates, em.kind[wv], em.out[wv], scratch + PFRAG / 2 + wv * (NCAT * NS), lane);
+    }
 }
 
 #ifdef PML_OPTIME
@@ -896,6 +912,10 @@
                 const NewtonReq &r = *reinterpret_cast<const NewtonReq *>(op.aux);
                 if (tid == 0 && blk == 0) { r.out[0] = r.t0; r.out[1] = __builtin_nan(""); r.out[2] = 0.0; r.out[3] = 0.0; }
             } else newton_fused(op, const_cast<double *>(buf), X, xsc, active, blk, ctl, timeout_ticks);
+#pragma unroll
+            for (int c = 0; c < 4; ++c)
+#pragma unroll
+                for (int k = 0; k < 5; ++k) X[c].v[k] = (dvec2){0.0, 0.0};
         }
 #ifdef PML_OPTIME
         const long long t_b0 = clock64(); t_newton += t_b0 - t_n0;
@@ -1270,6 +1290,14 @@
     if (per_request) hipExtLaunchKernelGGL(k_pmat<true>, dim3(blocks), dim3(PMAT_THREADS), 0, s, start, stop, 0, model, reqs, frags, n);
     else hipExtLaunchKernelGGL(k_pmat<false>, dim3(blocks), dim3(PMAT_THREADS), 0, s, start, stop, 0, model, reqs, frags, n);
 }
+void launch_pmat_to(const ModelDev *model, const PmatReq *reqs, double *const *outs, int n, hipStream_t s, bool per_request) {
+    if (n <= 0) return;
+    const int per_block = PMAT_THREADS / 64;
+    const int blocks = std::min((n + per_block - 1) / per_block, 512);
+    double *o = reinterpret_cast<double *>(const_cast<double **>(outs));
+    if (per_request) hipLaunchKernelGGL((k_pmat<true, true>), dim3(blocks), dim3(PMAT_THREADS), 0, s, model, reqs, o, n);
+    else hipLaunchKernelGGL((k_pmat<false, true>), dim3(blocks), dim3(PMAT_THREADS), 0, s, model, reqs, o, n);
+}
 void launch_eigfrags(const ModelDev *model, double *frags2, hipStream_t s) {
     hipLaunchKernelGGL(k_eigfrags, dim3(1), dim3(256), 0, s, model, frags2);
 }
```

After: 189.2. Within noise of the previous version (-0.5%).
